# NoSuchThingAsRandom/EpidemicSimulator

Hardware: AMD Instinct MI355X
Metric: citizen-timesteps/sec (higher is better)
Workload: dtype u32 citizen word; u32 uniform vs ceil(q*2^32) (reference: f64 uniform; tolerance 2^-32 per draw); 1 GPU; uk64m: 64000000 citizens, 290000 Output Areas, 10 seeds, steps 1..667 of 5000, interventions on; seed=1592598545

## Files before the change

### epidemicsimulator_amd/csrc/esim_device.h

```cpp
#pragma once
#include <stdint.h>

#define CW_TE_SHIFT    19u
#define CW_BUS_EXPOSED (1u << 18)
#define CW_FLAGS       0xFFu
#define CW_VAX_SHIFT   11u
#define CW_VAX_MASK    (0x7Fu << CW_VAX_SHIFT)
#define CW_KEEP        (CW_FLAGS | CW_VAX_MASK)
#define CW_VAX_NONE    0xFFFFFFFFu
#define CW_PLAN_SKIP   (1u << 10)
#define CW_VAX_REL(w)  ((((w) >> CW_VAX_SHIFT) & 0x7Fu) ? 127u - (((w) >> CW_VAX_SHIFT) & 0x7Fu) : CW_VAX_NONE)
#define CW_VAX_FIELD(j) ((127u - (j)) << CW_VAX_SHIFT)
#define CW_TE(w)       ((w) >> CW_TE_SHIFT)
#define CW_MAKE(te, rest) (((te) << CW_TE_SHIFT) | (rest))
#define TE_SUSCEPTIBLE 0x1FFFu
#define TE_VACCINATED  0x1FFEu
#define TE_RECOVERED   0x1FFDu
#define TE_BIAS        512u
#define TE_SLOTS       8192u
#define ESIM_MAX_STEP  7600u

#define FL_USES_PT        0x01u
#define FL_MASK_COMPLIANT 0x02u
#define FL_SAME_AREA      0x04u
#define FL_WORK_SCHOOL    0x08u
#define FL_HAS_WORK       0x10u
#define FL_BIG_ROUTE      0x20u

#define VACC_BATCH 4096u
#define VACC_WINDOW 32768u
#define VACC_TABLE 16384u
#define VACC_MAX_RATE 8192u
#define NO_ROUTE 0xFFFFFFFFu

#define MARK_SLOTS 4

struct Ctrl {
    uint32_t t;
    uint32_t lockdown;
    uint32_t mask;
    uint32_t vacc_active;
    uint32_t have_elig;
    uint32_t trigger_step;
    uint32_t elig_count;
    uint32_t finished;
    uint32_t stop_when_done;
    uint32_t at_work;
    uint32_t bus_dir;
    uint32_t steps_done;
    uint32_t error;
    uint32_t n_susceptible, n_vaccinated, n_recovered_sentinel;
    uint32_t log_len;
    uint32_t n_touched_bld[MARK_SLOTS], n_touched_room[MARK_SLOTS], n_touched_route[MARK_SLOTS], n_touched_route_big[MARK_SLOTS];
    uint32_t counts[5];
    uint32_t n_riders;
    uint32_t future_t0;
    uint32_t small_done;
    uint32_t chunk_ok;
    uint32_t chunk_t0;
    uint32_t chunk_i0, chunk_i1;
    uint32_t items_per_wave;
    uint32_t chunk_parallel;
    uint32_t chunk_pairs;
    uint32_t n_items;
    uint32_t n_newexp;
    uint32_t n_units, unit_next;
    uint32_t n_route_pairs_big;
    uint32_t chunk_done;
    uint32_t prev_t0, prev_n_items, prev_per_wave;
    uint32_t vax_chunk;
    uint32_t chunk_cut;
    uint32_t prev_cut;
    uint32_t prev_n, prev_n_eff, prev_vax;
    uint32_t vax_cuts;
    uint32_t vax_planned, prev_planned;
    uint32_t xs_need;
    uint32_t xs_need_all;
    uint32_t vax_fail;
    uint32_t err_where;
    uint32_t peer_error;
    uint32_t quiet;
    uint32_t chunk_bus;
    uint32_t replan_from;
    uint32_t repair_ran;
    uint32_t vax_repairs;
};

#define ERR_FIELD(code) ((code) ? 1u << (5u * (((code) < 1u || (code) > 6u ? 6u : (code)) - 1u)) : 0u)
#define ERR_MAX_WORLD 31u
#define XE_WORDS (2u + ERR_MAX_WORLD)
static inline __host__ __device__ uint32_t err_decode(uint32_t word)
{
    for (uint32_t c = 1u; c <= 6u; ++c) if ((word >> (5u * (c - 1u))) & 31u) return c;
    return word ? 6u : 0u;
}

struct UnitRec { uint32_t slot, link, lo, n_mem, code, own, m_first, pad; };

struct BldRec { uint32_t res_lo, res_hi, wrk_lo, wrk_hi, type, ovf_lo, ovf_hi, pad; };
#define SD_REPL 8u

struct ItemRec { uint32_t id, a_lo, a_hi, b_lo, b_hi, aux, link, own; };
#define CHUNK_WAVES_MAX 4096u
#define SLOT_COUNTERS_ONLY 0x40000000u
#ifndef ITEM_RECS
#define ITEM_RECS 7u
#define SLOT_IV_STRIDE 8u
#endif
#define LANE_STATE 24u
#define LANE_HSLOT 25u

struct Decision {
    uint32_t lockdown;
    uint32_t mask;
    uint32_t at_work, bus_dir;
};

struct Dev {
    uint32_t n;
    uint32_t n_global;
    uint32_t id_base;
    uint32_t n_bld, n_room, n_pt;
    uint32_t *cit;
    const uint32_t *home, *work, *room;
    const uint32_t *res_off, *res_idx;
    const uint32_t *wrk_off, *wrk_idx;
    const uint32_t *room_off, *room_idx;
    const uint32_t *room_bld;
    const uint8_t  *bld_type;
    uint32_t *cnt_bld[MARK_SLOTS];
    uint32_t *cnt_room[MARK_SLOTS];
    uint32_t *touched_bld[MARK_SLOTS], *touched_room[MARK_SLOTS], *touched_route[MARK_SLOTS], *touched_route_big[MARK_SLOTS];
    uint32_t *route_flag[MARK_SLOTS];
    uint32_t *exp_step;
    uint32_t *exp_part;
    struct Decision *dec;
    unsigned long long *hkey;
    uint32_t hcap;
    uint32_t *hitems;
    struct ItemRec *item_rec;
    uint32_t *slot_state;
    uint32_t *slot_iv;
    uint32_t *vec;
    uint32_t items_cap;
    struct UnitRec *units;
    uint32_t *route_pairs;
    uint32_t *pair_cnt;
    uint32_t *used_cnt;
    uint32_t *route_pairs_big;
    uint32_t big_pairs_cap;
    const uint32_t *ovf_off;
    uint32_t ovf_room_base;
    uint32_t *ovf;
    uint32_t ovf_n;
    uint32_t n_wrk_idx, n_room_idx;
    const int32_t *sch_of_bld;
    uint32_t n_sch;
    uint32_t *sch_diff;
    const uint4 *where4;
    const struct BldRec *bld8;
    uint32_t *big_list;
    uint32_t big_qcap;
    uint32_t *used_pref;
    uint32_t unit_qcap;
    uint32_t *newexp;
    uint32_t newexp_cap;
    uint32_t *hot;
    uint32_t *cursor;
    uint32_t max_route;
    uint32_t *vax_ev;
    uint32_t *vax_cnt;
    uint32_t *vax_now;
    uint32_t *lost_list;
    uint32_t *vax_delta;
    uint32_t *xf_adj;
    uint32_t *hist;
    uint32_t *log;
    uint32_t *log_off;
    const uint64_t *thr;
    Ctrl *ctrl;
    struct esim_step_result *records;
    uint32_t n_routes;
    const uint32_t *route_off;
    const uint32_t *route_riders;
    const uint32_t *route_of;
    uint32_t *bus_key; uint32_t *bus_idx; uint32_t *bus_cnt; uint8_t *bus_flag;
    uint32_t exposed_time, infected_time, vaccination_rate, bus_capacity, start_hour, end_hour;
    uint32_t seed_lo, seed_hi;
    double thr_lockdown, thr_vacc, thr_mask_pt, thr_mask_all;
    uint32_t max_steps;
    uint32_t n_shards;
    uint32_t n_shared_bld, n_shared_room;
    const int32_t *shared_bld, *shared_room;
    uint32_t *xa, *xb, *xf;
    uint32_t rank, world;
    uint32_t *xv;
    uint32_t *xs;
    uint32_t xs_cap;
    uint32_t *xs_out;
    const uint32_t *shared_mask;
    uint32_t *xc;
    uint32_t *xl;
    uint32_t *xe;
    const int32_t *shared_of_bld, *shared_of_room;
#ifdef ESIM_COUNT_WORK
    unsigned long long *work_cnt;
#endif
#ifdef ESIM_WAVE_PROFILE
    uint32_t *prof_buf;
#endif
    uint32_t xf_n;
    const uint32_t *bld_area;
    uint32_t n_areas;
};

#define XA_HEADER 8u
#define XB_HEADER 8u
#define FREE_MAX 96u
#define HKEY_EMPTY 0xFFFFFFFFFFFFFFFFull
#define PLAN_W 4096u
#define XV_HEADER 8u
#define XS_CAP_MAX (1u << 20)
#define HOT_STRIDE 32u
#define SUBQ 64u
#define HOT_NEWEXP 0u
#define HOT_UNITS 64u
#define HOT_BIGPAIRS 128u
#define HOT_BIG 129u
#define HOT_PREV_NEWEXP 257u
#define HOT_RESET 257u
#define HOT_LOST 321u
#define HOT_COUNT 322u
#define RAISE(ctrl, code, where) do { (ctrl)->error = (uint32_t)(-(code)); (ctrl)->err_where = (where); } while (0)
enum { ERR_AT_BIG_LIST = 2, ERR_AT_ITEM_CHECK = 6, ERR_AT_ROUTE_ITEM = 7, ERR_AT_BIGPAIRS = 10, ERR_AT_SCHOOL = 11 };
#define UNIT_NOOP 0xFFFFFFFFu
#ifndef LOST_CAP
#define LOST_CAP 8192u
#endif
#define CHUNK_BUS_STEPS 32u
#define PAIR_K(per_wave, nbus) ((per_wave) * ((nbus) > 8u ? ((nbus) + 3u) / 4u : 2u))
#define COUNT_GRID 256u
#define EXP_ROWS 32u
#ifndef UNIT_INLINE
#define UNIT_INLINE 1024u
#endif
#ifndef UNIT_PAIRS
#define UNIT_PAIRS 1024u
#endif
#define CHUNK_ROUTE_MAX 2048u
```

### epidemicsimulator_amd/csrc/esim_host_ctx.h

```cpp
namespace {

thread_local std::string g_create_error;

struct Timing {
    bool phase = false, kernel = false;
    uint32_t stride = 16;
    hipEvent_t ev[5] = { nullptr, nullptr, nullptr, nullptr, nullptr };
    double phase_s[3] = { 0, 0, 0 };
    std::vector<hipEvent_t> kev; size_t kev_used = 0;
    hipEvent_t cev[2] = { nullptr, nullptr }; double chunk_ms = 0; uint64_t chunk_steps = 0, chunk_count = 0;
    std::vector<hipEvent_t> pkev; size_t pkev_used = 0; uint64_t pipe_steps = 0;
    hipEvent_t sev[2] = { nullptr, nullptr }; double small_ms = 0; uint64_t small_steps = 0;
    bool kdetail = false;
    std::vector<hipEvent_t> kdev; std::vector<int> kd_kind; size_t kd_used = 0;
    double kd_ms[ESIM_CK_N] = { 0 }; uint64_t kd_calls[ESIM_CK_N] = { 0 };
    bool host_trace = false;
    std::vector<std::pair<const char *, double>> ht;

    static void make_pair(hipEvent_t (&e)[2]) { if (!e[0]) { (void)hipEventCreate(&e[0]); (void)hipEventCreate(&e[1]); } }
    void clear()
    {
        phase_s[0] = phase_s[1] = phase_s[2] = 0;
        kev_used = 0; pkev_used = 0; pipe_steps = 0;
        small_ms = 0; small_steps = 0; chunk_ms = 0; chunk_steps = 0; chunk_count = 0;
    }
    void destroy()
    {
        for (auto &e : ev) if (e) (void)hipEventDestroy(e);
        for (auto &e : cev) if (e) (void)hipEventDestroy(e);
        for (auto &e : sev) if (e) (void)hipEventDestroy(e);
        for (auto *v : { &kev, &pkev, &kdev }) { for (auto &e : *v) (void)hipEventDestroy(e); v->clear(); }
    }
};

struct Comm {
    int rank = 0, world = 1;
    ncclComm_t nccl = nullptr;
    esim_allreduce_fn fn = nullptr; void *user = nullptr;
    std::vector<uint32_t> stage;
    uint32_t *xr = nullptr; size_t xr_n = 0;
    uint64_t chunk_steps = 0, step_steps = 0;
    uint64_t calls = 0;
    double timeout_s = 60.0;
};

struct Pinned {
    Ctrl *ctrl = nullptr;
    esim_step_result *rec = nullptr; size_t rec_n = 0;
    uint32_t first = 0, valid = 0;
    bool track = false;
    bool ctrl_fresh = false;
    uint32_t *area = nullptr; size_t area_n = 0;
    uint32_t *grp = nullptr;
    uint8_t *aw = nullptr;
};

struct RestartStaging {
    uint32_t *seeds_dev = nullptr; size_t seeds_cap = 0;
    struct Block { Ctrl h; uint64_t lut[512]; } *stage = nullptr;
    uint32_t *seeds_stage = nullptr; size_t seeds_stage_n = 0;
    hipEvent_t ev = nullptr; bool ev_used = false;
};

struct Ensemble {
    uint32_t *hit = nullptr, *members = nullptr;
    unsigned long long *sum = nullptr, *sumsq = nullptr;
    int where = ESIM_AREA_HOME; uint32_t mask = 0, min = 0;
    bool arrival = false; uint32_t horizon = 0;
    uint32_t n = 0; bool valid = false;
    enum { ROWS_SERIES = 0, ROWS_SETTINGS = 1, ROWS_REPRODUCTION = 2 };
    struct Rows {
        uint32_t *hit = nullptr, *members = nullptr, *p0 = nullptr, *p1 = nullptr, *occ = nullptr, *vax = nullptr;
        unsigned long long *sum = nullptr, *sumsq = nullptr;
        uint8_t *aw = nullptr;
        int what = 0; uint32_t first = 0, n_rows = 0, stride = 0, min = 0, n_cols = 0;
        bool two = false;
        int kind = ROWS_SERIES;
        uint32_t mask = 0;
        uint32_t r_num = 0, r_den = 0;
        uint32_t *defined = nullptr;
        unsigned long long *sum_o = nullptr, *sumsq_o = nullptr, *cross = nullptr;
    } rows;
    bool series = false;
};

struct Groups {
    uint16_t *lab = nullptr; uint32_t n = 0;
    uint32_t *size = nullptr, *cnt = nullptr;
};

struct Snapshot {
    uint32_t step = 0;
    esim_params P;
    Ctrl h;
    uint32_t *words = nullptr, *hist = nullptr, *log_off = nullptr, *exp_step = nullptr;
    esim_step_result *records = nullptr;
    uint32_t *log = nullptr; size_t log_cap = 0;
    uint32_t last_chunk_pairs = 0; bool quiet = false, repair_armed = false, elig_seen = false;
    uint64_t vax_chunk_steps = 0, vax_chunk_cuts = 0, vax_chunk_repairs = 0;
};

struct Seam { uint32_t step = 0, rate = 0; uint64_t seed = 0; };

struct DrawSeam { uint32_t step = 0; bool twice = false, two_capacities = false; uint64_t seed = 0; double chance = 0.0, mask_effectiveness = 0.0; };

struct Tuning {
    uint32_t grid_citizens = 1, grid_infected = 1, grid_expose = 1;
    uint32_t grid_chunk = 1024;
    bool grid_chunk_env = false;
    bool pipeline = true;
    bool time_parallel = true;
    bool vax_chunks = true;
    bool vax_repair = true;
    bool vax_repair_always = false;
    uint32_t tiny_pairs = 2048;
    uint32_t small_grid = 64, small_mult = 4;
    uint32_t draw_mult = 4, units_mult = 4;
    uint32_t small_max = 128;
    uint32_t pair_log2 = 0;
};

struct PairStats {
    double ms[3] = { 0.0, 0.0, 0.0 };
    uint32_t distinct = 0, capacity = 0, dropped = 0;
};

struct esim_ctx_impl {
    esim_params P;
    Dev d;
    bool uploaded = false;
    hipStream_t stream = nullptr;
    std::string err;
    std::vector<uint32_t> init_state;
    std::vector<uint32_t> init_log;
    size_t cnt_bytes = 0;
    uint32_t *cnt_base = nullptr;
    uint32_t n_routes = 0;
    std::vector<uint32_t> route_tab;
    uint32_t longest_list = 0;
    size_t xa_n = 0, xb_n = 0, xf_n = 0;
    uint64_t pop_hash = 0;
    uint64_t pop_hash_head = 0;
    uint32_t cap_steps = 0;
    uint32_t *area_cnt = nullptr;
    uint32_t *arrival = nullptr;
    std::vector<void *> allocs;
    uint32_t host_t = 1;
    uint32_t last_chunk_pairs = 0;
    uint32_t stop_flag_dev = 0;
    bool quiet = false;
    bool repair_armed = false;
    bool elig_seen = false;
    uint32_t rest_t = 0;
    uint64_t vax_chunk_steps = 0, vax_chunk_cuts = 0, vax_chunk_repairs = 0;
    Timing tm;
    PairStats pair_stats;
    Comm comm;
    Pinned pin;
    RestartStaging rs;
    Ensemble ens;
    Groups grp;
    Snapshot snap;
    Seam seam;
    DrawSeam draw_seam;
    DrawSeam snap_draw_seam;
    Tuning tune;
};

#define CTX(c) (reinterpret_cast<esim_ctx_impl *>(c))

void comm_release(esim_ctx_impl *c);
int wait_stream(esim_ctx_impl *c);

int fail(esim_ctx_impl *c, int code, const std::string &msg)
{
    if (c) c->err = msg; else g_create_error = msg;
    return code;
}

#define HIP_TRY(c, expr)                                                                         \
    do {                                                                                         \
        hipError_t e_ = (expr);                                                                  \
        if (e_ != hipSuccess)                                                                    \
            return fail(c, ESIM_ENODEVICE, std::string(#expr) + ": " + hipGetErrorString(e_));   \
    } while (0)

int alloc_failed(esim_ctx_impl *c, hipError_t e) { return fail(c, ESIM_ENOMEM, std::string("hipMalloc: ") + hipGetErrorString(e)); }

template <class T> int dev_alloc(esim_ctx_impl *c, T **p, size_t n)
{
    void *q = nullptr;
    hipError_t e = hipMalloc(&q, sizeof(T) * (n ? n : 1));
    if (e != hipSuccess) return alloc_failed(c, e);
    c->allocs.push_back(q);
    *p = (T *)q;
    return ESIM_OK;
}

template <class T> int dev_alloc_fill(esim_ctx_impl *c, T **p, size_t n, int byte = 0)
{
    if (int rc = dev_alloc(c, p, n)) return rc;
    if (n) HIP_TRY(c, hipMemset(*p, byte, sizeof(T) * n));
    return ESIM_OK;
}

template <class T> int dev_upload(esim_ctx_impl *c, const T **p, const T *host, size_t n)
{
    T *q = nullptr;
    int rc = dev_alloc(c, &q, n);
    if (rc) return rc;
    if (n) HIP_TRY(c, hipMemcpy(q, host, sizeof(T) * n, hipMemcpyHostToDevice));
    *p = q;
    return ESIM_OK;
}

void free_device(esim_ctx_impl *c)
{
    for (void *p : c->allocs) (void)hipFree(p);
    c->allocs.clear();
    c->uploaded = false;
}

void dev_free(esim_ctx_impl *c, void *p)
{
    auto it = std::find(c->allocs.begin(), c->allocs.end(), p);
    if (it == c->allocs.end()) return;
    c->allocs.erase(it);
    (void)hipFree(p);
}

template <class T> struct DevTmp {
    T *p = nullptr;
    DevTmp() = default; DevTmp(const DevTmp &) = delete; DevTmp &operator=(const DevTmp &) = delete;
    ~DevTmp() { (void)hipFree(p); }
    hipError_t alloc(size_t n) { return hipMalloc((void **)&p, sizeof(T) * std::max<size_t>(1, n)); }
};

int drain(esim_ctx_impl *c) { HIP_TRY(c, hipSetDevice(c->P.device)); HIP_TRY(c, hipStreamSynchronize(c->stream)); return ESIM_OK; }

uint32_t grid_for(size_t items, uint32_t per_block, uint32_t cap)
{
    size_t g = (items + per_block - 1) / per_block;
    return (uint32_t)std::max<size_t>(1, std::min<size_t>(g, cap));
}

static inline void ht_mark(esim_ctx_impl *c, const char *what)
{
    if (!c->tm.host_trace) return;
    timespec ts; clock_gettime(CLOCK_MONOTONIC, &ts);
    c->tm.ht.emplace_back(what, ts.tv_sec * 1e6 + ts.tv_nsec * 1e-3);
}

int read_ctrl(esim_ctx_impl *c, Ctrl *h)
{
    HIP_TRY(c, hipMemcpyAsync(c->pin.ctrl, c->d.ctrl, sizeof(Ctrl), hipMemcpyDeviceToHost, c->stream));
    HIP_TRY(c, hipStreamSynchronize(c->stream));
    *h = *c->pin.ctrl;
    return ESIM_OK;
}

int ctrl_error(esim_ctx_impl *c, const Ctrl &h)
{
    if (!h.error) return ESIM_OK;
    const int code = -(int)(h.peer_error ? err_decode(h.peer_error) : h.error);
    return fail(c, code, "device-side error " + std::to_string(code) + " (S underflow / vaccination window exhausted / a chunk table check; raised at check " +
                         std::to_string(h.err_where) + ", esim_device.h ERR_AT_*)");
}

int device_error(esim_ctx_impl *c)
{
    Ctrl h;
    const int rc = read_ctrl(c, &h);
    return rc ? rc : ctrl_error(c, h);
}

}

extern "C" void esim_default_params(esim_params *p)
{
    if (!p) return;
    p->exposure_chance = 0.00055; p->mask_effectiveness = 0.70;
    p->lockdown_threshold = 0.0034; p->vaccination_threshold = 0.005;
    p->mask_pt_threshold = 0.001; p->mask_everywhere_threshold = 0.0022;
    p->exposed_time = 4 * 24; p->infected_time = 14 * 24;
    p->vaccination_rate = 85 * 18;
    p->bus_capacity = 20;
    p->start_hour = 9; p->end_hour = 17;
    p->seed = 0x5EED2011ull;
    p->device = 0;
    p->max_steps = 5000;
}

extern "C" int esim_threshold_lut(const esim_params *p, uint64_t out[512])
{
    if (!p || !out) return ESIM_EINVAL;
    for (int row = 0; row < 2; ++row) {
        double chance = p->exposure_chance - (row ? p->exposure_chance * p->mask_effectiveness : 0.0) - 0.0;
        if (std::signbit(chance)) chance = 0.0;
        for (int n = 0; n < 256; ++n) {
            const double q = 1.0 - std::pow(1.0 - chance, (double)n);
            const double scaled = std::ceil(std::ldexp(q, 32));
            out[row * 256 + n] = scaled <= 0.0 ? 0ull : (uint64_t)scaled;
        }
    }
    return ESIM_OK;
}

namespace {
int check_params(esim_ctx_impl *c, const esim_params *p, const std::string &who)
{
    if (p->exposed_time + p->infected_time + 2u > TE_BIAS)
        return fail(c, ESIM_ERANGE, who + ": exposed_time + infected_time + 2 exceeds the state encoding (512)");
    if (p->vaccination_rate > VACC_MAX_RATE)
        return fail(c, ESIM_ERANGE, who + ": vaccination_rate above 8192 is not supported");
    if (p->bus_capacity == 0 || p->start_hour == 0 || p->end_hour == 0 || p->start_hour > 24 || p->end_hour > 24)
        return fail(c, ESIM_EINVAL, who + ": bad bus_capacity / working hours");
    {
        const uint32_t h[4] = { (p->start_hour + 23u) % 24u, p->start_hour % 24u, (p->end_hour + 23u) % 24u, p->end_hour % 24u };
        for (int a = 0; a < 4; ++a) for (int b = a + 1; b < 4; ++b)
            if (h[a] == h[b]) return fail(c, ESIM_EINVAL, who + ": start_hour-1, start_hour, end_hour-1, end_hour must be distinct");
        if (p->start_hour > 23 || p->end_hour > 23) return fail(c, ESIM_EINVAL, who + ": working hours must be in 1..23");
    }
    if (p->max_steps == 0 || p->max_steps > ESIM_MAX_STEP)
        return fail(c, ESIM_ERANGE, who + ": max_steps must be in 1..7600");
    if (!(p->exposure_chance >= 0.0 && p->exposure_chance <= 1.0))
        return fail(c, ESIM_EINVAL, who + ": exposure_chance must be a probability");
    return ESIM_OK;
}

void params_to_dev(esim_ctx_impl *c)
{
    Dev &d = c->d;
    d.exposed_time = c->P.exposed_time; d.infected_time = c->P.infected_time;
    d.vaccination_rate = c->P.vaccination_rate; d.bus_capacity = c->P.bus_capacity;
    d.start_hour = c->P.start_hour; d.end_hour = c->P.end_hour;
    d.seed_lo = (uint32_t)c->P.seed; d.seed_hi = (uint32_t)(c->P.seed >> 32);
    d.thr_lockdown = c->P.lockdown_threshold; d.thr_vacc = c->P.vaccination_threshold;
    d.thr_mask_pt = c->P.mask_pt_threshold; d.thr_mask_all = c->P.mask_everywhere_threshold;
    d.max_steps = c->P.max_steps;
    c->xf_n =std::min<uint32_t>(FREE_MAX, c->P.exposed_time + 1u);
    d.xf_n = (uint32_t)c->xf_n;
}
}

extern "C" int esim_create(const esim_params *p, esim_ctx **out)
{
    if (!p || !out) return fail(nullptr, ESIM_EINVAL, "esim_create: null argument");
    if (int rc = check_params(nullptr, p, "esim_create")) return rc;
    int n_dev = 0;
    hipError_t e = hipGetDeviceCount(&n_dev);
    if (e != hipSuccess || n_dev <= 0)
        return fail(nullptr, ESIM_ENODEVICE, std::string("esim_create: no HIP device (") + hipGetErrorString(e) + ")");
    if (p->device < 0 || p->device >= n_dev) return fail(nullptr, ESIM_EINVAL, "esim_create: device ordinal out of range");
    e = hipSetDevice(p->device);
    if (e != hipSuccess) return fail(nullptr, ESIM_ENODEVICE, std::string("hipSetDevice: ") + hipGetErrorString(e));
    esim_ctx_impl *c = new esim_ctx_impl();
    c->P = *p;
    c->cap_steps = p->max_steps;
    if (const char *e = std::getenv("ESIM_COMM_TIMEOUT_S")) { const double v = std::atof(e); if (v > 0.0) c->comm.timeout_s = v; }
    std::memset(&c->d, 0, sizeof c->d);
    e = hipStreamCreateWithFlags(&c->stream, hipStreamNonBlocking);
    if (e != hipSuccess) { delete c; return fail(nullptr, ESIM_ENODEVICE, std::string("hipStreamCreate: ") + hipGetErrorString(e)); }
    for (auto &ev : c->tm.ev) (void)hipEventCreate(&ev);
    *out = reinterpret_cast<esim_ctx *>(c);
    return ESIM_OK;
}

extern "C" void esim_destroy(esim_ctx *ctx)
{
    if (ctx) comm_release(CTX(ctx));
    if (!ctx) return;
    esim_ctx_impl *c = CTX(ctx);
    (void)hipSetDevice(c->P.device);
    if (c->stream) (void)hipStreamSynchronize(c->stream);
    free_device(c);
    c->tm.destroy();
    for (void *p : { (void *)c->pin.ctrl, (void *)c->pin.rec, (void *)c->pin.area, (void *)c->pin.grp, (void *)c->pin.aw, (void *)c->rs.stage, (void *)c->rs.seeds_stage })
        if (p) (void)hipHostFree(p);
    if (c->rs.ev) (void)hipEventDestroy(c->rs.ev);
    if (c->stream) (void)hipStreamDestroy(c->stream);
    delete c;
}

extern "C" const char *esim_last_error(const esim_ctx *ctx)
{
    if (!ctx) return g_create_error.c_str();
    return reinterpret_cast<const esim_ctx_impl *>(ctx)->err.c_str();
}
```

### epidemicsimulator_amd/csrc/esim_host_run.h

```cpp
namespace {

int enqueue_begin(esim_ctx_impl *c, bool time_kernel)
{
    Dev &d = c->d;
    if (c->tm.phase) HIP_TRY(c, hipEventRecord(c->tm.ev[0], c->stream));
    if (time_kernel) HIP_TRY(c, hipEventRecord(c->tm.kev[c->tm.kev_used + 0], c->stream));
    hipLaunchKernelGGL(k_infected, dim3(c->tune.grid_infected), dim3(TPB), 0, c->stream, d);
    if (d.n_shards > 1) {
        const uint32_t n = (uint32_t)std::max<size_t>(XA_HEADER, std::max(d.n_shared_bld, d.n_shared_room));
        hipLaunchKernelGGL(k_pack_a, dim3(grid_for(n, TPB, 1u << 20)), dim3(TPB), 0, c->stream, d);
    }
    if (c->tm.phase) HIP_TRY(c, hipEventRecord(c->tm.ev[1], c->stream));
    return ESIM_OK;
}

int enqueue_exposures(esim_ctx_impl *c)
{
    Dev &d = c->d;
    if (d.n_shards > 1) {
        const uint32_t n = (uint32_t)std::max<size_t>(XA_HEADER, std::max(d.n_shared_bld, d.n_shared_room));
        hipLaunchKernelGGL(k_unpack_a, dim3(grid_for(n, TPB, 1u << 20)), dim3(TPB), 0, c->stream, d);
    }
    hipLaunchKernelGGL(k_expose, dim3(c->tune.grid_expose), dim3(TPB), 0, c->stream, d);
    if (d.n_shards > 1) hipLaunchKernelGGL(k_pack_b, dim3(VACC_WINDOW / TPB), dim3(TPB), 0, c->stream, d);
    if (c->tm.phase) HIP_TRY(c, hipEventRecord(c->tm.ev[2], c->stream));
    return ESIM_OK;
}

int enqueue_finish(esim_ctx_impl *c, bool time_kernel, int mode = -1)
{
    Dev &d = c->d;
    if (mode < 0) mode = d.n_shards > 1 ? 1 : 0;
    hipLaunchKernelGGL(k_finish, dim3(1), dim3(FIN_TPB), 0, c->stream, d, mode);
    if (time_kernel) { HIP_TRY(c, hipEventRecord(c->tm.kev[c->tm.kev_used + 1], c->stream)); c->tm.kev_used += 2; }
    if (c->tm.phase) {
        HIP_TRY(c, hipEventRecord(c->tm.ev[3], c->stream));
        HIP_TRY(c, hipEventSynchronize(c->tm.ev[3]));
        float ms;
        for (int i = 0; i < 3; ++i) { HIP_TRY(c, hipEventElapsedTime(&ms, c->tm.ev[i], c->tm.ev[i + 1])); c->tm.phase_s[i] += ms * 1e-3; }
    }
    c->host_t++;
    HIP_TRY(c, hipGetLastError());
    return ESIM_OK;
}

int check_budget(esim_ctx_impl *c, uint32_t n_steps)
{
    if (!c || !c->uploaded) return fail(c, ESIM_ESTATE, "no population uploaded");
    if ((uint64_t)c->host_t + n_steps - 1 > c->P.max_steps)
        return fail(c, ESIM_ERANGE, "step budget exhausted: max_steps reached (DiseaseModel::max_time_step)");
    return ESIM_OK;
}

bool want_kernel_timing(esim_ctx_impl *c)
{
    Timing &t = c->tm;
    if (!t.kernel || (c->host_t % t.stride) != 0) return false;
    if (t.kev_used + 2 > t.kev.size()) {
        for (int i = 0; i < 2; ++i) { hipEvent_t e; if (hipEventCreate(&e) != hipSuccess) return false; t.kev.push_back(e); }
    }
    return true;
}

void kd_mark(esim_ctx_impl *c, int kind)
{
    Timing &t = c->tm;
    if (!t.kdetail) return;
    if (t.kd_used == t.kdev.size()) { hipEvent_t e; if (hipEventCreate(&e) != hipSuccess) return; t.kdev.push_back(e); t.kd_kind.push_back(0); }
    if (hipEventRecord(t.kdev[t.kd_used], c->stream) != hipSuccess) return;
    t.kd_kind[t.kd_used++] = kind;
}

void kd_resolve(esim_ctx_impl *c)
{
    Timing &t = c->tm;
    for (size_t i = 0; i + 1 < t.kd_used; ++i) {
        if (t.kd_kind[i] >= ESIM_CK_N) continue;
        float ms = 0.f;
        if (hipEventElapsedTime(&ms, t.kdev[i], t.kdev[i + 1]) == hipSuccess) { t.kd_ms[t.kd_kind[i]] += ms; t.kd_calls[t.kd_kind[i]]++; }
    }
    t.kd_used = 0;
}

int chunk_time_begin(esim_ctx_impl *c) { if (c->tm.kernel) { Timing::make_pair(c->tm.cev); HIP_TRY(c, hipEventRecord(c->tm.cev[0], c->stream)); } return ESIM_OK; }
int chunk_time_end(esim_ctx_impl *c) { if (c->tm.kernel) HIP_TRY(c, hipEventRecord(c->tm.cev[1], c->stream)); return ESIM_OK; }

int burst_readback(esim_ctx_impl *c, uint32_t first, uint32_t span, Ctrl *h)
{
    const Dev &d = c->d;
    Pinned &pin = c->pin;
    ht_mark(c, "kernels enqueued");
    HIP_TRY(c, hipMemcpyAsync(pin.ctrl, d.ctrl, sizeof(Ctrl), hipMemcpyDeviceToHost, c->stream));
    const bool rec = pin.track && first == pin.first + pin.valid && (size_t)first + span <= pin.rec_n;
    if (rec) HIP_TRY(c, hipMemcpyAsync(pin.rec + first, d.records + first, sizeof(esim_step_result) * span, hipMemcpyDeviceToHost, c->stream));
    ht_mark(c, "copies enqueued");
    HIP_TRY(c, hipStreamSynchronize(c->stream));
    ht_mark(c, "stream drained");
    *h = *pin.ctrl;
    if (rec && h->t >= first) pin.valid += std::min<uint32_t>(h->t - first, span);
    pin.ctrl_fresh = true;
    if (c->tm.kdetail) kd_resolve(c);
    return ESIM_OK;
}

int run_sequential(esim_ctx_impl *c, uint32_t n_steps, bool allow_early_stop, uint32_t *executed)
{
    Dev &d = c->d; Timing &t = c->tm;
    c->pin.ctrl_fresh = false;
    c->quiet = false;
    uint32_t remaining = n_steps, total = 0; int rc;
    const bool persistent = c->tune.small_max > 0 && !t.phase;
    while (remaining > 0) {
        if (persistent) {
            if (t.kernel) { Timing::make_pair(t.sev); HIP_TRY(c, hipEventRecord(t.sev[0], c->stream)); }
            hipLaunchKernelGGL(k_small, dim3(1), dim3(FIN_TPB), 0, c->stream, d, remaining, c->tune.small_max, 0);
            if (t.kernel) HIP_TRY(c, hipEventRecord(t.sev[1], c->stream));
            Ctrl h;
            if ((rc = read_ctrl(c, &h))) return rc;
            if (t.kernel && h.small_done) { float ms; HIP_TRY(c, hipEventElapsedTime(&ms, t.sev[0], t.sev[1])); t.small_ms += ms; t.small_steps += h.small_done; }
            c->host_t += h.small_done; total += h.small_done; remaining -= h.small_done;
            if ((rc = ctrl_error(c, h))) return rc;
            if (h.finished && allow_early_stop) break;
        }
        if (remaining == 0) break;
        const uint32_t chunk = std::min<uint32_t>(remaining, persistent ? 32u : remaining);
        for (uint32_t s = 0; s < chunk; ++s) {
            const bool tk = want_kernel_timing(c);
            if ((rc = enqueue_begin(c, tk))) return rc;
            if ((rc = enqueue_exposures(c))) return rc;
            if ((rc = enqueue_finish(c, tk, 0))) return rc;
        }
        total += chunk; remaining -= chunk;
    }
    if (executed) *executed = total;
    return ESIM_OK;
}

bool tiny_chunk(const esim_ctx_impl *c) { return c->tune.tiny_pairs && c->last_chunk_pairs <= c->tune.tiny_pairs && c->d.world == 1u && c->d.n_shards == 1u; }
bool small_chunk(const esim_ctx_impl *c) { return c->tune.small_grid && c->last_chunk_pairs < 4096u && c->tune.grid_chunk > c->tune.small_grid && !c->tune.grid_chunk_env; }

struct ChunkPass {
    esim_ctx_impl *c;
    uint32_t limit_t;
    bool kd;
    uint32_t n_ahead() const { return (uint32_t)c->xf_n; }
    void mark(int kind) const { if (kd) kd_mark(c, kind); }
    void future(uint32_t n) const { mark(ESIM_CK_FUTURE); hipLaunchKernelGGL(k_future, dim3(1), dim3(FIN_TPB), 0, c->stream, c->d, n, limit_t); }
    void decide(uint32_t n, int parallel, int vax_in_census) const { mark(ESIM_CK_DECIDE); hipLaunchKernelGGL(k_decide, dim3(1), dim3(64), 0, c->stream, c->d, n, limit_t, parallel, vax_in_census); }
    void vax_plan(int sharded) const { mark(ESIM_CK_VAX); hipLaunchKernelGGL(k_chunk_vax<false>, dim3(FREE_MAX + (sharded ? 0u : 1u)), dim3(FIN_TPB), 0, c->stream, c->d, n_ahead(), limit_t, sharded); }
    void lost() const { mark(ESIM_CK_VAX_REPAIR); hipLaunchKernelGGL(k_chunk_lost, dim3(1), dim3(FIN_TPB), 0, c->stream, c->d); }
    void vax_repair(int sharded) const { hipLaunchKernelGGL(k_chunk_vax<true>, dim3(FREE_MAX), dim3(FIN_TPB), 0, c->stream, c->d, n_ahead(), limit_t, sharded); }
    void front(bool few) const
    {
        const Tuning &t = c->tune;
        const uint32_t g = few ? t.small_grid : t.grid_chunk, g_draw = g * (few ? t.small_mult : t.draw_mult), g_units = g * (few ? t.small_mult : t.units_mult);
        mark(ESIM_CK_MARKS); hipLaunchKernelGGL(k_chunk_marks, dim3(g), dim3(TPB), 0, c->stream, c->d);
        mark(ESIM_CK_FOLD); hipLaunchKernelGGL(k_chunk_fold, dim3(g), dim3(TPB), 0, c->stream, c->d);
        mark(ESIM_CK_DRAW); hipLaunchKernelGGL(k_chunk_draw, dim3(g_draw), dim3(TPB), 0, c->stream, c->d, g * (TPB / 64u));
        mark(ESIM_CK_UNITS); hipLaunchKernelGGL(k_chunk_units, dim3(g_units), dim3(TPB), 0, c->stream, c->d);
    }
    void count() const { mark(ESIM_CK_COUNT); hipLaunchKernelGGL(k_chunk_count, dim3(COUNT_GRID), dim3(TPB), 0, c->stream, c->d); }
    void scatter() const { mark(ESIM_CK_SCATTER); hipLaunchKernelGGL(k_chunk_scatter, dim3(COUNT_GRID), dim3(TPB), 0, c->stream, c->d); }
    void books(int alone, int then_next) const { mark(ESIM_CK_BOOKS); hipLaunchKernelGGL(k_chunk_books, dim3(1), dim3(FIN_TPB), 0, c->stream, c->d, alone, then_next, n_ahead(), limit_t); }
    void vax_final() const { mark(ESIM_CK_VAX_FINAL); hipLaunchKernelGGL(k_chunk_vax_final, dim3(FREE_MAX), dim3(TPB), 0, c->stream, c->d); }
};

void enqueue_parallel_chunk(esim_ctx_impl *c, int then_next, uint32_t limit_t)
{
    const ChunkPass p{ c, limit_t, true };
    const bool alone = c->last_chunk_pairs < 1024u;
    p.front(small_chunk(c));
    if (!alone) p.count();
    p.books(alone ? 1 : 0, then_next);
    if (!alone) p.scatter();
    p.mark(ESIM_CK_N);
}

void enqueue_vax_chunk(esim_ctx_impl *c, uint32_t limit_t)
{
    const ChunkPass p{ c, limit_t, true };
    const Tuning &t = c->tune;
    const bool quiet = c->quiet && c->d.world == 1u;
    p.vax_plan(0);
    p.decide(p.n_ahead(), 1, 0);
    if (!quiet) {
        p.front(small_chunk(c));
        if (c->d.world == 1u && t.vax_repair && (c->repair_armed || t.vax_repair_always)) { p.lost(); p.vax_repair(0); }
    }
    p.count();
    p.books(0, 0);
    if (!quiet) p.scatter();
    p.vax_final();
    p.mark(ESIM_CK_N);
}

void enqueue_free_burst(esim_ctx_impl *c, uint32_t bursts, uint32_t limit_t)
{
    const ChunkPass p{ c, limit_t, true };
    if (tiny_chunk(c)) {
        for (uint32_t g = 0; g < bursts; ++g) {
            p.mark(ESIM_CK_TINY);
            hipLaunchKernelGGL(k_chunk_tiny, dim3(1), dim3(FIN_TPB), 0, c->stream, c->d, g == 0u ? 1 : 0, g + 1u < bursts ? 1 : 0, p.n_ahead(), limit_t);
        }
        p.mark(ESIM_CK_N);
        return;
    }
    p.future(p.n_ahead());
    p.decide(p.n_ahead(), 1, 0);
    for (uint32_t g = 0; g < bursts; ++g) enqueue_parallel_chunk(c, g + 1u < bursts ? 1 : 0, limit_t);
}

int run_chunk(esim_ctx_impl *c, uint32_t n_ahead, uint32_t *executed, Ctrl *state_before)
{
    Dev &d = c->d; Timing &t = c->tm;
    c->pin.ctrl_fresh = false;
    ChunkPass{ c, c->P.max_steps, false }.decide(n_ahead, c->tune.time_parallel ? 1 : 0, 0);
    Ctrl h; int rc;
    if ((rc = read_ctrl(c, &h))) return rc;
    *state_before = h;
    if ((rc = ctrl_error(c, h))) return rc;
    const uint32_t n = h.chunk_ok, t0 = h.t;
    c->last_chunk_pairs = h.chunk_pairs;
    *executed = 0;
    if (n == 0) return ESIM_OK;
    if (h.chunk_parallel) {
        if ((rc = chunk_time_begin(c))) return rc;
        enqueue_parallel_chunk(c, 0, 0u);
        if ((rc = chunk_time_end(c))) return rc;
        if (t.kernel) { float ms; HIP_TRY(c, hipEventSynchronize(t.cev[1])); HIP_TRY(c, hipEventElapsedTime(&ms, t.cev[0], t.cev[1])); t.chunk_ms += ms; }
        HIP_TRY(c, hipGetLastError());
        Ctrl after;
        if ((rc = read_ctrl(c, &after)) || (rc = ctrl_error(c, after))) return rc;
        const uint32_t ran = after.t - t0;
        t.chunk_steps += ran; t.chunk_count += ran ? 1u : 0u;
        *executed = ran;
        return ESIM_OK;
    }
    hipLaunchKernelGGL(k_infected_dec, dim3(c->tune.grid_infected), dim3(TPB), 0, c->stream, d, t0, 0u);
    for (uint32_t j = 0; j < n; ++j) {
        bool tk = t.kernel && ((t0 + j) % t.stride) == 0;
        if (tk && t.pkev_used + 2 > t.pkev.size())
            for (int i = 0; i < 2 && tk; ++i) { hipEvent_t e; if (hipEventCreate(&e) != hipSuccess) tk = false; else t.pkev.push_back(e); }
        if (tk) HIP_TRY(c, hipEventRecord(t.pkev[t.pkev_used], c->stream));
        hipLaunchKernelGGL(k_pipe, dim3(c->tune.grid_expose + c->tune.grid_infected), dim3(TPB), 0, c->stream, d, t0 + j, j, c->tune.grid_expose, j + 1 < n ? 1 : 0);
        if (tk) { HIP_TRY(c, hipEventRecord(t.pkev[t.pkev_used + 1], c->stream)); t.pkev_used += 2; }
    }
    hipLaunchKernelGGL(k_batch_finish, dim3(1), dim3(FIN_TPB), 0, c->stream, d, t0, n);
    HIP_TRY(c, hipGetLastError());
    t.pipe_steps += n;
    *executed = n;
    return ESIM_OK;
}

int run_burst(esim_ctx_impl *c, uint32_t remaining, uint32_t bursts, bool vax, Ctrl *h, uint32_t *done)
{
    const uint32_t first = c->host_t, limit_t = first + remaining - 1u, n_ahead = (uint32_t)c->xf_n;
    int rc;
    if ((rc = chunk_time_begin(c))) return rc;
    if (!vax) enqueue_free_burst(c, bursts, limit_t);
    else for (uint32_t g = 0; g < bursts; ++g) enqueue_vax_chunk(c, limit_t);
    if ((rc = chunk_time_end(c))) return rc;
    if ((rc = burst_readback(c, first, std::min<uint32_t>(remaining, bursts * n_ahead), h))) return rc;
    HIP_TRY(c, hipGetLastError());
    if ((rc = ctrl_error(c, *h))) return rc;
    *done = h->t - first;
    c->last_chunk_pairs = h->chunk_pairs;
    Timing &t = c->tm;
    if (*done && t.kernel) { float ms; HIP_TRY(c, hipEventElapsedTime(&ms, t.cev[0], t.cev[1])); t.chunk_ms += ms; t.chunk_steps += *done; t.chunk_count += (*done + n_ahead - 1u) / n_ahead; }
    c->host_t = h->t;
    return ESIM_OK;
}

int run_steps(esim_ctx_impl *c, uint32_t n_steps, bool allow_early_stop, uint32_t *executed)
{
    Dev &d = c->d;
    const uint32_t n_ahead_max = (uint32_t)c->xf_n;
    uint32_t remaining = n_steps, total = 0; int rc;
    bool stalled = false, probing = false;
    uint32_t backoff = 0, sync_chunks_left = 0;
    const bool vax_ok = c->tune.time_parallel && c->tune.vax_chunks && d.n_shards == 1u;
    bool sequential_only = !c->tune.pipeline || c->tm.phase, vax_regime = vax_ok && c->elig_seen;
    if (c->elig_seen && (!vax_ok || n_steps < 8u)) sequential_only = true;
    auto programme_started = [&]() { c->elig_seen = true; if (vax_ok && remaining >= 8u) vax_regime = true; else sequential_only = true; };
    uint32_t vax_fail = 0;
    while (remaining > 0) {
        c->pin.ctrl_fresh = false;
        if (sequential_only) {
            uint32_t done = 0;
            if ((rc = run_sequential(c, remaining, allow_early_stop, &done))) return rc;
            total += done;
            break;
        }
        if (vax_regime) {
            const uint32_t bursts = vax_fail ? 1u : std::min<uint32_t>((remaining + n_ahead_max - 1u) / n_ahead_max + 1u, 8u);
            Ctrl h;
            uint32_t done = 0;
            if ((rc = run_burst(c, remaining, bursts, true, &h, &done))) return rc;
            c->quiet = h.quiet != 0u;
            if (h.vax_cuts > c->vax_chunk_cuts) c->repair_armed = true;
            c->vax_chunk_steps += done; c->vax_chunk_cuts = h.vax_cuts; c->vax_chunk_repairs = h.vax_repairs;
            total += done; remaining -= done;
            if (h.finished && allow_early_stop) break;
            if (remaining == 0) break;
            if (done) { vax_fail = 0; continue; }
            if (std::getenv("ESIM_DEBUG"))
                std::fprintf(stderr, "[esim] vax burst without progress at t=%u: chunk_ok=%u parallel=%u vax_chunk=%u cut=%u pairs=%u fits_flag=%u elig=%u bursts=%u\n",
                             h.t, h.chunk_ok, h.chunk_parallel, h.vax_chunk, h.chunk_cut, h.chunk_pairs, 0u, h.elig_count, bursts);
            vax_fail = std::min<uint32_t>(vax_fail + 1u, 8u);
            uint32_t seq = 0;
            const uint32_t want = std::min<uint32_t>(remaining, vax_fail <= 1u ? 1u : (vax_fail <= 3u ? 8u : n_ahead_max));
            if ((rc = run_sequential(c, want, allow_early_stop, &seq))) return rc;
            total += seq; remaining -= seq;
            if (seq < want) break;
            continue;
        }
        if (c->tune.time_parallel && !stalled && sync_chunks_left == 0) {
            const uint32_t bursts = std::min<uint32_t>((remaining + n_ahead_max - 1u) / n_ahead_max, probing ? 1u : (small_chunk(c) ? 4u : 16u));
            Ctrl h;
            uint32_t done = 0;
            if ((rc = run_burst(c, remaining, bursts, false, &h, &done))) return rc;
            total += done; remaining -= done;
            if (h.finished) break;
            const bool all = done >= std::min<uint32_t>(remaining + done, bursts * n_ahead_max);
            if (done == 0) { backoff = std::min<uint32_t>(64u, backoff ? backoff * 2u : 1u); sync_chunks_left = backoff; probing = true; }
            else { backoff = 0; probing = !all; }
            if (!all) stalled = true;
            continue;
        }
        stalled = false;
        if (sync_chunks_left) --sync_chunks_left;
        const uint32_t n_ahead = std::min<uint32_t>(remaining, n_ahead_max);
        ChunkPass{ c, c->P.max_steps, false }.future(n_ahead);
        uint32_t done = 0;
        Ctrl before;
        if ((rc = run_chunk(c, n_ahead, &done, &before))) return rc;
        c->host_t = before.t + done; total += done; remaining -= done;
        if (before.finished) break;
        if (done < n_ahead && remaining > 0) {
            if (before.have_elig || before.vacc_active) { programme_started(); continue; }
            uint32_t one = 0;
            if ((rc = run_sequential(c, 1, allow_early_stop, &one))) return rc;
            total += one; remaining -= one;
            if (one == 0) break;
            Ctrl h;
            if ((rc = read_ctrl(c, &h))) return rc;
            if (h.have_elig) programme_started();
        }
        if (allow_early_stop && done > 0) {
            Ctrl h;
            if ((rc = read_ctrl(c, &h))) return rc;
            if (h.finished) { c->host_t = h.t; break; }
        }
    }
    if (executed) *executed = total;
    return ESIM_OK;
}

}

extern "C" int esim_step(esim_ctx *ctx, esim_step_result *out)
{
    esim_ctx_impl *c = CTX(ctx);
    int rc = check_budget(c, 1);
    if (rc) return rc;
    if (c->d.n_shards > 1) return fail(c, ESIM_ESTATE, "esim_step: a sharded population runs with esim_run_sharded");
    HIP_TRY(c, hipSetDevice(c->P.device));
    c->rest_t = 0;
    if ((rc = run_steps(c, 1, false, nullptr))) return rc;
    HIP_TRY(c, hipStreamSynchronize(c->stream));
    if (out) HIP_TRY(c, hipMemcpy(out, &c->d.records[c->host_t - 1], sizeof *out, hipMemcpyDeviceToHost));
    if ((rc = device_error(c))) return rc;
    c->rest_t = c->host_t;
    return ESIM_OK;
}

extern "C" int esim_run(esim_ctx *ctx, uint32_t n_steps, int stop_when_done, esim_step_result *out_array, uint32_t *n_done)
{
    esim_ctx_impl *c = CTX(ctx);
    if (c && c->tm.host_trace) { c->tm.ht.clear(); ht_mark(c, "enter"); }
    int rc = check_budget(c, n_steps);
    if (rc) return rc;
    if (c->d.n_shards > 1) return fail(c, ESIM_ESTATE, "esim_run: a sharded population runs with esim_run_sharded");
    HIP_TRY(c, hipSetDevice(c->P.device));
    Pinned &pin = c->pin;
    const uint32_t first = c->host_t;
    const uint32_t flag = stop_when_done ? 1u : 0u;
    if (flag != c->stop_flag_dev) {
        HIP_TRY(c, hipMemcpyAsync(&c->d.ctrl->stop_when_done, &flag, sizeof flag, hipMemcpyHostToDevice, c->stream));
        HIP_TRY(c, hipStreamSynchronize(c->stream));
        c->stop_flag_dev = flag;
    }
    pin.track = out_array != nullptr; pin.first = first; pin.valid = 0; pin.ctrl_fresh = false;
    c->rest_t = 0;
    rc = run_steps(c, n_steps, stop_when_done != 0, nullptr);
    pin.track = false;
    if (rc) return rc;
    Ctrl h;
    if (pin.ctrl_fresh) h = *pin.ctrl;
    else if ((rc = read_ctrl(c, &h))) return rc;
    if ((rc = ctrl_error(c, h))) return rc;
    const uint32_t done = h.steps_done >= first ? h.steps_done - first + 1 : 0;
    if (std::getenv("ESIM_DEBUG"))
        std::fprintf(stderr, "[esim] esim_run(%u steps from %u): done %u, t=%u steps_done=%u finished=%u chunk_ok=%u parallel=%u, records mirrored %u, control block %s\n",
                     n_steps, first, done, h.t, h.steps_done, h.finished, h.chunk_ok, h.chunk_parallel, pin.valid, pin.ctrl_fresh ? "from the burst" : "read now");
    c->host_t = first + done;
    c->rest_t = c->host_t;
    if (out_array && done) {
        const uint32_t have = std::min(pin.valid, done);
        if (have < done) {
            HIP_TRY(c, hipMemcpyAsync(pin.rec + first + have, c->d.records + first + have, sizeof(esim_step_result) * (done - have), hipMemcpyDeviceToHost, c->stream));
            HIP_TRY(c, hipStreamSynchronize(c->stream));
        }
        std::memcpy(out_array, pin.rec + first, sizeof(esim_step_result) * done);
    }
    if (n_done) *n_done = done;
    if (c->tm.host_trace) {
        ht_mark(c, "exit");
        std::fprintf(stderr, "[esim host trace] esim_run(%u):", n_steps);
        for (size_t i = 1; i < c->tm.ht.size(); ++i) std::fprintf(stderr, " %s +%.1f us;", c->tm.ht[i].first, c->tm.ht[i].second - c->tm.ht[i - 1].second);
        std::fprintf(stderr, " total %.1f us\n", c->tm.ht.back().second - c->tm.ht.front().second);
    }
    return ESIM_OK;
}

extern "C" int esim_set_pipeline(esim_ctx *ctx, int enable)
{
    esim_ctx_impl *c = CTX(ctx); if (!c) return ESIM_EINVAL;
    c->tune.pipeline = enable != 0;
    c->tune.time_parallel = enable >= 2;
    c->tune.vax_chunks = enable >= 3;
    return ESIM_OK;
}

extern "C" int esim_set_small_step_limit(esim_ctx *ctx, uint32_t max_infected)
{
    esim_ctx_impl *c = CTX(ctx); if (!c) return ESIM_EINVAL;
    c->tune.small_max = max_infected;
    return ESIM_OK;
}

extern "C" int esim_set_tiny_chunk_limit(esim_ctx *ctx, uint32_t max_pairs)
{
    esim_ctx_impl *c = CTX(ctx); if (!c) return ESIM_EINVAL;
    c->tune.tiny_pairs = max_pairs;
    return ESIM_OK;
}
```

### epidemicsimulator_amd/csrc/esim_host_upload.h

```cpp
namespace {

struct UploadHost {
    const esim_population *pop;
    uint32_t N, B, R, n_global;
    bool sharded;
    std::vector<uint8_t> fl;
    std::vector<uint32_t> room_fixed;
    std::vector<uint32_t> route_off, riders, route_of;
    uint32_t n_routes = 0, max_route = 0, n_big_routes = 0;
    bool any_big = false;
    std::vector<uint32_t> res_off, res_idx, wrk_off, wrk_idx, room_off, room_idx;
    bool home_sorted = true;
};

int upload_validate(esim_ctx_impl *c, UploadHost &u)
{
    const esim_population *pop = u.pop; const uint32_t N = u.N, B = u.B, R = u.R;
    if (!pop->home_building || !pop->work_building || !pop->room || !pop->flags || !pop->building_area || !pop->building_type)
        return fail(c, ESIM_EINVAL, "esim_upload_population: a required array is NULL");
    if (R && !pop->room_building) return fail(c, ESIM_EINVAL, "esim_upload_population: room_building is NULL");
    if (pop->n_seeds && !pop->seeds) return fail(c, ESIM_EINVAL, "esim_upload_population: seeds is NULL");
    u.n_global = pop->n_citizens_global ? pop->n_citizens_global : N;
    if ((uint64_t)pop->citizen_id_base + N > u.n_global) return fail(c, ESIM_EINVAL, "esim_upload_population: shard range exceeds n_citizens_global");
    u.sharded = u.n_global != N || pop->n_shared_buildings || pop->n_shared_rooms;
    u.fl.resize(N);
    for (uint32_t b = 0; b < B; ++b) {
        if (pop->building_area[b] >= pop->n_areas) return fail(c, ESIM_EINVAL, "esim_upload_population: building_area out of range");
        if (pop->building_type[b] > ESIM_SCHOOL) return fail(c, ESIM_EINVAL, "esim_upload_population: unknown building_type");
    }
    for (uint32_t r = 0; r < R; ++r)
        if (pop->room_building[r] >= B || pop->building_type[pop->room_building[r]] != ESIM_SCHOOL)
            return fail(c, ESIM_EINVAL, "esim_upload_population: room_building must name a School");
    u.room_fixed.assign(N, 0);
    for (uint32_t i = 0; i < N; ++i) {
        const uint32_t hb = pop->home_building[i], wb = pop->work_building[i];
        if (hb >= B || wb >= B) return fail(c, ESIM_EINVAL, "esim_upload_population: building index out of range");
        if (pop->building_type[hb] == ESIM_SCHOOL) return fail(c, ESIM_EINVAL, "esim_upload_population: a School cannot be a home");
        uint8_t f = pop->flags[i] & (FL_USES_PT | FL_MASK_COMPLIANT);
        if (pop->building_area[hb] == pop->building_area[wb]) f |= FL_SAME_AREA;
        if (hb != wb) {
            f |= FL_HAS_WORK;
            if (pop->building_type[wb] == ESIM_SCHOOL) {
                f |= FL_WORK_SCHOOL;
                if (pop->room[i] >= R || pop->room_building[pop->room[i]] != wb)
                    return fail(c, ESIM_EINVAL, "esim_upload_population: school member without a room of that school");
                u.room_fixed[i] = pop->room[i];
            }
        }
        u.fl[i] = f;
    }
    for (uint32_t i = 0; i < pop->n_seeds; ++i)
        if (pop->seeds[i] >= N) return fail(c, ESIM_EINVAL, "esim_upload_population: seed index out of range");
    for (uint32_t i = 0; i < pop->n_shared_buildings; ++i)
        if (pop->shared_building_local[i] >= (int32_t)B) return fail(c, ESIM_EINVAL, "esim_upload_population: shared building out of range");
    for (uint32_t i = 0; i < pop->n_shared_rooms; ++i)
        if (pop->shared_room_local[i] >= (int32_t)R) return fail(c, ESIM_EINVAL, "esim_upload_population: shared room out of range");
    return ESIM_OK;
}

void fnv_mix(uint64_t &h, const void *p, size_t nbytes)
{
    const uint8_t *q = (const uint8_t *)p;
    for (size_t i = 0; i < nbytes; ++i) { h ^= q[i]; h *= 0x100000001b3ull; }
}

uint64_t hash_with_seeds(uint64_t head, const uint32_t *seeds, uint32_t n_seeds)
{
    if (n_seeds) fnv_mix(head, seeds, sizeof(uint32_t) * (size_t)n_seeds);
    return head;
}

uint64_t population_hash(const esim_population *pop, uint64_t *head)
{
    const size_t N = pop->n_citizens, B = pop->n_buildings, R = pop->n_rooms;
    uint64_t h = 0xcbf29ce484222325ull;
    fnv_mix(h, pop->home_building, sizeof(uint32_t) * N); fnv_mix(h, pop->work_building, sizeof(uint32_t) * N);
    fnv_mix(h, pop->room, sizeof(uint32_t) * N); fnv_mix(h, pop->flags, N);
    fnv_mix(h, pop->building_area, sizeof(uint32_t) * B); fnv_mix(h, pop->building_type, B);
    if (R) fnv_mix(h, pop->room_building, sizeof(uint32_t) * R);
    *head = h;
    return hash_with_seeds(h, pop->seeds, pop->n_seeds);
}

void upload_routes(UploadHost &u)
{
    const esim_population *pop = u.pop;
    std::vector<std::pair<uint64_t, uint32_t>> pairs;
    for (uint32_t i = 0; i < u.N; ++i)
        if (u.fl[i] & FL_USES_PT)
            pairs.emplace_back(((uint64_t)pop->building_area[pop->home_building[i]] << 32) | pop->building_area[pop->work_building[i]], i);
    std::sort(pairs.begin(), pairs.end());
    u.riders.resize(pairs.size()); u.route_of.assign(u.N, NO_ROUTE);
    for (size_t i = 0; i < pairs.size(); ++i) {
        if (i == 0 || pairs[i].first != pairs[i - 1].first) u.route_off.push_back((uint32_t)i);
        u.riders[i] = pairs[i].second;
        u.route_of[pairs[i].second] = (uint32_t)u.route_off.size() - 1;
    }
    u.n_routes = (uint32_t)u.route_off.size();
    u.route_off.push_back((uint32_t)pairs.size());
    for (uint32_t r = 0; r < u.n_routes; ++r) {
        const uint32_t sz = u.route_off[r + 1] - u.route_off[r];
        u.max_route = std::max(u.max_route, sz);
        if (sz > 64) { u.any_big = true; ++u.n_big_routes; for (uint32_t q = u.route_off[r]; q < u.route_off[r + 1]; ++q) u.fl[u.riders[q]] |= FL_BIG_ROUTE; }
    }
}

void upload_member_lists(UploadHost &u)
{
    const esim_population *pop = u.pop;
    const std::vector<uint8_t> &fl = u.fl;
    auto csr = [](uint32_t n_keys, uint32_t n_items, auto key_of, auto use, std::vector<uint32_t> &off, std::vector<uint32_t> &idx) {
        off.assign((size_t)n_keys + 1, 0);
        for (uint32_t i = 0; i < n_items; ++i) if (use(i)) off[key_of(i) + 1]++;
        for (uint32_t k = 0; k < n_keys; ++k) off[k + 1] += off[k];
        idx.resize(off[n_keys]);
        std::vector<uint32_t> cur(off.begin(), off.end() - 1);
        for (uint32_t i = 0; i < n_items; ++i) if (use(i)) idx[cur[key_of(i)]++] = i;
    };
    csr(u.B, u.N, [&](uint32_t i) { return pop->home_building[i]; }, [&](uint32_t) { return true; }, u.res_off, u.res_idx);
    for (uint32_t i = 0; i < u.N && u.home_sorted; ++i) u.home_sorted = u.res_idx[i] == i;
    csr(u.B, u.N, [&](uint32_t i) { return pop->work_building[i]; },
        [&](uint32_t i) { return (fl[i] & FL_HAS_WORK) && !(fl[i] & FL_WORK_SCHOOL); }, u.wrk_off, u.wrk_idx);
    csr(u.R, u.N, [&](uint32_t i) { return u.room_fixed[i]; }, [&](uint32_t i) { return (fl[i] & FL_WORK_SCHOOL) != 0; }, u.room_off, u.room_idx);
}

uint32_t seed_te(const esim_ctx_impl *c) { return TE_BIAS - (c->P.exposed_time + 1u); }

int upload_population_tables(esim_ctx_impl *c, const UploadHost &u)
{
    const esim_population *pop = u.pop; const uint32_t N = u.N, B = u.B, R = u.R;
    comm_release(c);
    c->comm.fn = nullptr; c->comm.user = nullptr; c->comm.rank = 0; c->comm.world = 1;
    c->comm.xr = nullptr; c->comm.xr_n = 0;
    free_device(c);
    c->rs.seeds_dev = nullptr; c->rs.seeds_cap = 0;
    c->arrival = nullptr;
    c->ens.hit = c->ens.members = nullptr; c->ens.sum = c->ens.sumsq = nullptr;
    c->ens.rows = Ensemble::Rows(); c->ens.series = false;
    c->ens.valid = false;
    c->grp = Groups();
    c->snap = Snapshot();
    Dev &d = c->d;
    std::memset(&d, 0, sizeof d);
    d.n = N; d.n_global = u.n_global; d.id_base = pop->citizen_id_base; d.n_bld = B; d.n_room = R;
    d.n_pt = (uint32_t)u.riders.size(); d.n_routes = u.n_routes; c->n_routes = u.n_routes;
    d.max_route = u.max_route;
    c->route_tab.assign(3 * (size_t)u.n_routes, 0u);
    for (uint32_t r = 0; r < u.n_routes; ++r) {
        const uint32_t first = u.riders[u.route_off[r]];
        c->route_tab[r] = pop->building_area[pop->home_building[first]];
        c->route_tab[u.n_routes + r] = pop->building_area[pop->work_building[first]];
        c->route_tab[2 * (size_t)u.n_routes + r] = u.route_off[r + 1] - u.route_off[r];
    }
    int rc;
    if ((rc = dev_alloc(c, &d.cit, (size_t)N + 1))) return rc;
    if ((rc = dev_upload(c, &d.home, pop->home_building, N)) || (rc = dev_upload(c, &d.work, pop->work_building, N))) return rc;
    if ((rc = dev_upload(c, &d.room, u.room_fixed.data(), N))) return rc;
    if ((rc = dev_upload(c, &d.res_off, u.res_off.data(), u.res_off.size()))) return rc;
    if (!u.home_sorted) { if ((rc = dev_upload(c, &d.res_idx, u.res_idx.data(), u.res_idx.size()))) return rc; }
    else d.res_idx = nullptr;
    if ((rc = dev_upload(c, &d.wrk_off, u.wrk_off.data(), u.wrk_off.size())) || (rc = dev_upload(c, &d.wrk_idx, u.wrk_idx.data(), u.wrk_idx.size()))) return rc;
    if ((rc = dev_upload(c, &d.room_off, u.room_off.data(), u.room_off.size())) || (rc = dev_upload(c, &d.room_idx, u.room_idx.data(), u.room_idx.size()))) return rc;
    if ((rc = dev_upload(c, &d.room_bld, pop->room_building, R))) return rc;
    if ((rc = dev_upload(c, &d.bld_type, pop->building_type, B))) return rc;
    if ((rc = dev_upload(c, &d.bld_area, pop->building_area, B))) return rc;
    d.n_areas = pop->n_areas;
    if ((rc = dev_alloc(c, &c->area_cnt, (size_t)pop->n_areas * 5u))) return rc;
    const size_t per_parity = (size_t)B + R + u.n_routes;
    if ((rc = dev_alloc(c, &c->cnt_base, MARK_SLOTS * per_parity))) return rc;
    c->cnt_bytes = sizeof(uint32_t) * MARK_SLOTS * per_parity;
    if ((rc = dev_alloc(c, &d.exp_step, 2 * ((size_t)c->cap_steps + 2)))) return rc;
    if ((rc = dev_alloc_fill(c, &d.exp_part, (size_t)EXP_ROWS * 2u * FREE_MAX))) return rc;
    if ((rc = dev_alloc(c, &d.dec, FREE_MAX + 1))) return rc;
    return ESIM_OK;
}

int upload_chunk_tables(esim_ctx_impl *c, const UploadHost &u)
{
    const esim_population *pop = u.pop; const uint32_t N = u.N, B = u.B;
    Dev &d = c->d; int rc;
    uint32_t cap = 1u << 20;
    while (cap < (1u << 26) && cap < N / 2u) cap <<= 1;
    if (const char *e = std::getenv("ESIM_HASH_LOG2")) cap = 1u << std::min(28, std::max(4, std::atoi(e)));
    d.hcap = cap;
    d.items_cap = cap / 4u;
    if ((rc = dev_alloc_fill(c, &d.hkey, cap, 0xFF))) return rc;
    if ((rc = dev_alloc_fill(c, &d.hitems, d.items_cap, 0xFF))) return rc;
    if ((rc = dev_alloc_fill(c, &d.item_rec, d.items_cap))) return rc;
    if ((rc = dev_alloc_fill(c, &d.vec, (size_t)cap * FREE_MAX))) return rc;
    if ((rc = dev_alloc_fill(c, &d.slot_state, cap))) return rc;
    if ((rc = dev_alloc_fill(c, &d.slot_iv, (size_t)cap * SLOT_IV_STRIDE))) return rc;
    size_t units = 0;
    auto add_lists = [&](const std::vector<uint32_t> &off) {
        for (size_t i = 0; i + 1 < off.size(); ++i) {
            const size_t pairs = (size_t)(off[i + 1] - off[i]) * FREE_MAX;
            if (pairs > UNIT_INLINE) units += (pairs + UNIT_PAIRS - 1) / UNIT_PAIRS;
        }
    };
    add_lists(u.res_off); add_lists(u.wrk_off); add_lists(u.room_off);
    units = std::min<size_t>(units, (size_t)N / 8u + 65536u);
    d.unit_qcap = (uint32_t)std::max<size_t>(1024, units * 2u / SUBQ);
    if ((rc = dev_alloc_fill(c, &d.units, (size_t)d.unit_qcap * SUBQ, 0xFF))) return rc;
    if ((rc = dev_alloc_fill(c, &d.route_pairs, (size_t)d.items_cap * (CHUNK_BUS_STEPS / 4u)))) return rc;
    d.big_pairs_cap = (uint32_t)std::max<size_t>(1, std::min<size_t>((size_t)d.items_cap / 4u, u.n_big_routes) * CHUNK_BUS_STEPS);
    if ((rc = dev_alloc_fill(c, &d.route_pairs_big, d.big_pairs_cap))) return rc;
    std::vector<uint32_t> sch_members((size_t)B + 1, 0);
    for (uint32_t i = 0; i < N; ++i) if (u.fl[i] & FL_WORK_SCHOOL) sch_members[pop->work_building[i] + 1]++;
    for (uint32_t b = 0; b < B; ++b) sch_members[b + 1] += sch_members[b];
    std::vector<uint32_t> ovf_off(u.res_off.size());
    for (size_t i = 0; i < u.res_off.size(); ++i) ovf_off[i] = u.res_off[i] + u.wrk_off[i] + sch_members[i];
    if ((rc = dev_upload(c, &d.ovf_off, ovf_off.data(), ovf_off.size()))) return rc;
    c->longest_list = u.max_route;
    for (const std::vector<uint32_t> *off : { &u.res_off, &u.wrk_off, &u.room_off })
        for (size_t i = 1; i < off->size(); ++i) c->longest_list = std::max(c->longest_list, (*off)[i] - (*off)[i - 1]);
    {
        std::vector<int32_t> sch_of(B ? B : 1, -1);
        uint32_t n_sch = 0;
        for (uint32_t b = 0; b < B; ++b) if (pop->building_type[b] == ESIM_SCHOOL) sch_of[b] = (int32_t)n_sch++;
        d.n_sch = n_sch;
        if ((rc = dev_upload(c, &d.sch_of_bld, sch_of.data(), sch_of.size()))) return rc;
    }
    {
        std::vector<uint4> w4(N ? N : 1);
        for (uint32_t i = 0; i < N; ++i) w4[i] = make_uint4(pop->home_building[i], pop->work_building[i], u.room_fixed[i], u.route_of[i]);
        if ((rc = dev_upload(c, &d.where4, w4.data(), w4.size()))) return rc;
        std::vector<BldRec> b8(B ? B : 1);
        for (uint32_t b = 0; b < B; ++b) b8[b] = BldRec{ u.res_off[b], u.res_off[b + 1], u.wrk_off[b], u.wrk_off[b + 1], (uint32_t)pop->building_type[b], ovf_off[b], ovf_off[b + 1], 0u };
        if ((rc = dev_upload(c, &d.bld8, b8.data(), b8.size()))) return rc;
        if ((rc = dev_alloc_fill(c, &d.sch_diff, (size_t)(d.n_sch ? d.n_sch : 1) * SD_REPL * 2u * FREE_MAX))) return rc;
    }
    d.ovf_room_base = ovf_off.back();
    d.ovf_n = d.ovf_room_base + u.room_off.back() + 1u;
    if ((rc = dev_alloc_fill(c, &d.ovf, (size_t)d.ovf_n))) return rc;
    d.n_wrk_idx = (uint32_t)u.wrk_idx.size(); d.n_room_idx = (uint32_t)u.room_idx.size();
    d.big_qcap = d.items_cap / SUBQ;
    if ((rc = dev_alloc_fill(c, &d.big_list, (size_t)d.big_qcap * SUBQ * 3u))) return rc;
    if ((rc = dev_alloc_fill(c, &d.used_pref, CHUNK_WAVES_MAX + 1u))) return rc;
    if ((rc = dev_alloc_fill(c, &d.pair_cnt, 16384u)) || (rc = dev_alloc_fill(c, &d.used_cnt, 16384u))) return rc;
    if ((rc = dev_alloc_fill(c, &d.hot, (size_t)HOT_COUNT * HOT_STRIDE))) return rc;
    d.newexp_cap = N / SUBQ + 1u;
    if ((rc = dev_alloc_fill(c, &d.newexp, (size_t)d.newexp_cap * SUBQ))) return rc;
    if ((rc = dev_alloc_fill(c, &d.cursor, (size_t)EXP_ROWS * FREE_MAX))) return rc;
    return ESIM_OK;
}

int upload_step_tables(esim_ctx_impl *c, const UploadHost &u)
{
    const uint32_t N = u.N, B = u.B, R = u.R;
    Dev &d = c->d; int rc;
    const size_t per_parity = (size_t)B + R + u.n_routes;
    for (int p = 0; p < (int)MARK_SLOTS; ++p) {
        uint32_t *base = c->cnt_base + p * per_parity;
        d.cnt_bld[p] = base; d.cnt_room[p] = base + B; d.route_flag[p] = base + B + R;
        if ((rc = dev_alloc(c, &d.touched_bld[p], B)) || (rc = dev_alloc(c, &d.touched_room[p], R))) return rc;
        if ((rc = dev_alloc(c, &d.touched_route[p], u.n_routes)) || (rc = dev_alloc(c, &d.touched_route_big[p], u.n_routes))) return rc;
    }
    if ((rc = dev_alloc(c, &d.vax_ev, (size_t)FREE_MAX * VACC_MAX_RATE))) return rc;
    if ((rc = dev_alloc_fill(c, &d.vax_cnt, FREE_MAX)) || (rc = dev_alloc_fill(c, &d.vax_now, FREE_MAX))) return rc;
    if ((rc = dev_alloc_fill(c, &d.vax_delta, 4u * (FREE_MAX + 2u)))) return rc;
    if ((rc = dev_alloc_fill(c, &d.lost_list, LOST_CAP))) return rc;
    if ((rc = dev_alloc_fill(c, &d.xf_adj, FREE_MAX + 2u))) return rc;
    if ((rc = dev_alloc(c, &d.hist, TE_SLOTS)) || (rc = dev_alloc(c, &d.log, (size_t)N + 1)) || (rc = dev_alloc(c, &d.log_off, TE_SLOTS + 1))) return rc;
    {
        const uint32_t *sd = nullptr;
        if ((rc = dev_upload(c, &sd, c->init_log.data(), c->init_log.size()))) return rc;
        c->rs.seeds_dev = const_cast<uint32_t *>(sd); c->rs.seeds_cap = c->init_log.size();
    }
    uint64_t lut[512];
    esim_threshold_lut(&c->P, lut);
    if ((rc = dev_upload(c, &d.thr, lut, 512))) return rc;
    if ((rc = dev_alloc(c, &d.ctrl, 1))) return rc;
    if ((rc = dev_alloc(c, &d.records, (size_t)c->cap_steps + 1))) return rc;
    if ((rc = dev_upload(c, &d.route_off, u.route_off.data(), u.route_off.size())) || (rc = dev_upload(c, &d.route_riders, u.riders.data(), u.riders.size()))) return rc;
    if ((rc = dev_upload(c, &d.route_of, u.route_of.data(), N))) return rc;
    const size_t big_scratch = u.any_big ? u.riders.size() : 0;
    if ((rc = dev_alloc(c, &d.bus_key, big_scratch)) || (rc = dev_alloc(c, &d.bus_idx, big_scratch))) return rc;
    if ((rc = dev_alloc(c, &d.bus_cnt, big_scratch)) || (rc = dev_alloc(c, &d.bus_flag, big_scratch))) return rc;
    params_to_dev(c);
    return ESIM_OK;
}

int upload_shard_tables(esim_ctx_impl *c, const UploadHost &u)
{
    const esim_population *pop = u.pop; const uint32_t B = u.B, R = u.R;
    Dev &d = c->d; int rc;
    d.n_shards = u.sharded ? 2u : 1u;
    d.n_shared_bld = pop->n_shared_buildings; d.n_shared_room = pop->n_shared_rooms;
    if ((rc = dev_upload(c, &d.shared_bld, pop->shared_building_local, pop->n_shared_buildings)) || (rc = dev_upload(c, &d.shared_room, pop->shared_room_local, pop->n_shared_rooms))) return rc;
    std::vector<int32_t> of_b(B ? B : 1, -1), of_r(R ? R : 1, -1);
    for (uint32_t i = 0; i < pop->n_shared_buildings; ++i) if (pop->shared_building_local[i] >= 0) of_b[pop->shared_building_local[i]] = (int32_t)i;
    for (uint32_t i = 0; i < pop->n_shared_rooms; ++i) if (pop->shared_room_local[i] >= 0) of_r[pop->shared_room_local[i]] = (int32_t)i;
    if ((rc = dev_upload(c, &d.shared_of_bld, of_b.data(), of_b.size())) || (rc = dev_upload(c, &d.shared_of_room, of_r.data(), of_r.size()))) return rc;
    if ((rc = dev_alloc_fill(c, &d.xv, XV_HEADER + (size_t)FREE_MAX * (PLAN_W / 32u)))) return rc;
    if ((rc = dev_alloc_fill(c, &d.xc, FREE_MAX + 2u)) || (rc = dev_alloc_fill(c, &d.xl, FREE_MAX + 2u)) || (rc = dev_alloc_fill(c, &d.xe, XE_WORDS))) return rc;
    d.rank = 0; d.world = 1; d.xs = nullptr;
#ifdef ESIM_COUNT_WORK
    if ((rc = dev_alloc_fill(c, &d.work_cnt, (size_t)WK_N))) return rc;
#endif
#ifdef ESIM_WAVE_PROFILE
    if ((rc = dev_alloc_fill(c, &d.prof_buf, (size_t)16384 * 16))) return rc;
#endif
    c->xa_n = XA_HEADER + (size_t)d.n_shared_bld + d.n_shared_room;
    c->xb_n = XB_HEADER + VACC_WINDOW / 32u;
    if ((rc = dev_alloc_fill(c, &d.xa, c->xa_n)) || (rc = dev_alloc_fill(c, &d.xb, c->xb_n)) || (rc = dev_alloc_fill(c, &d.xf, FREE_MAX + 1))) return rc;
    return ESIM_OK;
}

template <class T> int pinned_grow(esim_ctx_impl *c, T **p, size_t *have, size_t want)
{
    if (*have >= want) return ESIM_OK;
    if (*p) (void)hipHostFree(*p);
    *p = nullptr; *have = 0;
    HIP_TRY(c, hipHostMalloc((void **)p, sizeof(T) * std::max<size_t>(1, want), hipHostMallocDefault));
    *have = want;
    return ESIM_OK;
}

int upload_pinned(esim_ctx_impl *c, const UploadHost &u)
{
    if (!c->pin.ctrl) HIP_TRY(c, hipHostMalloc((void **)&c->pin.ctrl, sizeof(Ctrl), hipHostMallocDefault));
    if (!c->rs.stage) HIP_TRY(c, hipHostMalloc((void **)&c->rs.stage, sizeof(*c->rs.stage), hipHostMallocDefault));
    if (!c->rs.ev) HIP_TRY(c, hipEventCreateWithFlags(&c->rs.ev, hipEventDisableTiming));
    if (int rc = pinned_grow(c, &c->pin.rec, &c->pin.rec_n, (size_t)c->cap_steps + 1)) return rc;
    return pinned_grow(c, &c->pin.area, &c->pin.area_n, (size_t)u.pop->n_areas * 5u);
}

void upload_tuning(esim_ctx_impl *c, const UploadHost &u)
{
    Tuning &t = c->tune;
    t.grid_citizens = grid_for(u.N, TPB, 2048);
    t.grid_infected = 1024;
    t.grid_expose = 1024;
    if (const char *e = std::getenv("ESIM_GRID_INFECTED")) t.grid_infected = (uint32_t)std::max(1, std::atoi(e));
    const char *gc = std::getenv("ESIM_GRID_CHUNK");
    t.grid_chunk_env = gc != nullptr;
    if (gc) t.grid_chunk = (uint32_t)std::min((int)(CHUNK_WAVES_MAX * 64u / TPB), std::max(16, std::atoi(gc) / 16 * 16));
    if (std::getenv("ESIM_TRACE_HOST")) c->tm.host_trace = true;
    if (const char *e = std::getenv("ESIM_VAX_REPAIR")) { t.vax_repair = std::atoi(e) != 0; t.vax_repair_always = std::atoi(e) >= 2; }
    if (const char *e = std::getenv("ESIM_TINY_PAIRS")) t.tiny_pairs = (uint32_t)std::max(0, std::atoi(e));
    if (const char *e = std::getenv("ESIM_SMALL_GRID")) t.small_grid = (uint32_t)std::max(0, std::atoi(e) / 16 * 16);
    if (const char *e = std::getenv("ESIM_SMALL_MULT")) t.small_mult = (uint32_t)std::min(16, std::max(1, std::atoi(e)));
    if (const char *e = std::getenv("ESIM_DRAW_MULT")) t.draw_mult = (uint32_t)std::min(4, std::max(1, std::atoi(e)));
    if (const char *e = std::getenv("ESIM_UNITS_MULT")) t.units_mult = (uint32_t)std::min(16, std::max(1, std::atoi(e)));
    if (const char *e = std::getenv("ESIM_GRID_EXPOSE")) t.grid_expose = (uint32_t)std::max(1, std::atoi(e));
    t.pair_log2 = 0u;
    if (const char *e = std::getenv("ESIM_PAIR_LOG2")) t.pair_log2 = (uint32_t)std::min(31, std::max(6, std::atoi(e)));
}

}

extern "C" int esim_upload_population(esim_ctx *ctx, const esim_population *pop)
{
    esim_ctx_impl *c = CTX(ctx);
    if (!c || !pop) return fail(c, ESIM_EINVAL, "esim_upload_population: null argument");
    HIP_TRY(c, hipSetDevice(c->P.device));
    UploadHost u;
    u.pop = pop; u.N = pop->n_citizens; u.B = pop->n_buildings; u.R = pop->n_rooms;
    int rc;
    if ((rc = upload_validate(c, u))) return rc;
    c->pop_hash = population_hash(pop, &c->pop_hash_head);
    upload_routes(u);
    upload_member_lists(u);
    c->init_state.resize(u.N);
    for (uint32_t i = 0; i < u.N; ++i) c->init_state[i] = CW_MAKE(TE_SUSCEPTIBLE, (uint32_t)u.fl[i]);
    c->init_log.clear();
    for (uint32_t i = 0; i < pop->n_seeds; ++i) {
        const uint32_t sc = pop->seeds[i];
        if (CW_TE(c->init_state[sc]) != seed_te(c)) { c->init_state[sc] = CW_MAKE(seed_te(c), (uint32_t)u.fl[sc]); c->init_log.push_back(sc); }
    }
    if ((rc = upload_population_tables(c, u))) return rc;
    if ((rc = upload_chunk_tables(c, u))) return rc;
    if ((rc = upload_step_tables(c, u))) return rc;
    if ((rc = upload_shard_tables(c, u))) return rc;
    if ((rc = upload_pinned(c, u))) return rc;
    upload_tuning(c, u);
    c->uploaded = true;
    return esim_reset(ctx);
}

namespace {

void initial_ctrl(const esim_ctx_impl *c, Ctrl *h)
{
    const uint32_t n_seeds = (uint32_t)c->init_log.size();
    std::memset(h, 0, sizeof *h);
    h->t = 1;
    h->mask = ESIM_MASK_NONE;
    h->n_susceptible = c->d.n - n_seeds;
    h->log_len = n_seeds;
}

void rewind_host(esim_ctx_impl *c)
{
    c->host_t = 1;
    c->stop_flag_dev = 0;
    c->last_chunk_pairs = (uint32_t)c->init_log.size();
    c->vax_chunk_steps = 0; c->vax_chunk_cuts = 0; c->elig_seen = false; c->repair_armed = false; c->quiet = false;
    c->pin.track = false; c->pin.ctrl_fresh = false;
    c->rest_t = 0;
    c->seam = Seam();
    c->draw_seam = DrawSeam();
    c->tm.clear();
}

}

extern "C" int esim_reset(esim_ctx *ctx)
{
    esim_ctx_impl *c = CTX(ctx);
    if (!c || !c->uploaded) return fail(c, ESIM_ESTATE, "esim_reset: no population uploaded");
    if (int rc = drain(c)) return rc;
    const Dev &d = c->d;
    const uint32_t n_seeds = (uint32_t)c->init_log.size();
    Ctrl h;
    initial_ctrl(c, &h);
    HIP_TRY(c, hipMemcpy(d.ctrl, &h, sizeof h, hipMemcpyHostToDevice));
    if (d.n) HIP_TRY(c, hipMemcpy(d.cit, c->init_state.data(), sizeof(uint32_t) * (size_t)d.n, hipMemcpyHostToDevice));
    HIP_TRY(c, hipMemset(c->cnt_base, 0, c->cnt_bytes));
    HIP_TRY(c, hipMemset(d.exp_step, 0, sizeof(uint32_t) * 2 * ((size_t)c->P.max_steps + 2)));
    HIP_TRY(c, hipMemset(d.records, 0, sizeof(esim_step_result) * ((size_t)c->P.max_steps + 1)));
    const uint32_t te = seed_te(c);
    std::vector<uint32_t> hist(TE_SLOTS, 0), off(TE_SLOTS + 1, 0);
    hist[te] = n_seeds;
    for (uint32_t k = te + 1; k <= TE_SLOTS; ++k) off[k] = n_seeds;
    HIP_TRY(c, hipMemcpy(d.hist, hist.data(), sizeof(uint32_t) * TE_SLOTS, hipMemcpyHostToDevice));
    HIP_TRY(c, hipMemcpy(d.log_off, off.data(), sizeof(uint32_t) * (TE_SLOTS + 1), hipMemcpyHostToDevice));
    if (n_seeds) HIP_TRY(c, hipMemcpy(d.log, c->init_log.data(), sizeof(uint32_t) * n_seeds, hipMemcpyHostToDevice));
    rewind_host(c);
    return ESIM_OK;
}

namespace {

int restart_check(esim_ctx_impl *c, const esim_params *p, const std::string &who)
{
    if (!c->uploaded) return fail(c, ESIM_ESTATE, who + ": no population uploaded");
    if (c->comm.world > 1) return fail(c, ESIM_ESTATE, who + ": the context has a communicator of several ranks (the shards would have to agree on the parameters)");
    if (int rc = check_params(c, p, who)) return rc;
    if (p->device != c->P.device) return fail(c, ESIM_EINVAL, who + ": device must be the context's device");
    if (p->max_steps > c->cap_steps) return fail(c, ESIM_ERANGE, who + ": max_steps above the max_steps the context was created with (the record log's capacity)");
    return ESIM_OK;
}

int restart_enqueue(esim_ctx_impl *c, const esim_params *p, bool replace, const uint32_t *seeds, uint32_t n_seeds)
{
    HIP_TRY(c, hipSetDevice(c->P.device));
    if (c->rs.ev_used) HIP_TRY(c, hipEventSynchronize(c->rs.ev));
    if (replace) {
        if (int rc = pinned_grow(c, &c->rs.seeds_stage, &c->rs.seeds_stage_n, n_seeds)) return rc;
        if (n_seeds > c->rs.seeds_cap) {
            uint32_t *grown = nullptr;
            if (int rc = dev_alloc(c, &grown, n_seeds)) return rc;
            dev_free(c, c->rs.seeds_dev);
            c->rs.seeds_dev = grown; c->rs.seeds_cap = n_seeds;
        }
    }
    c->P = *p;
    params_to_dev(c);
    const Dev &d = c->d;
    const uint32_t te = seed_te(c);
    if (replace) {
        for (uint32_t sc : c->init_log) c->init_state[sc] = CW_MAKE(TE_SUSCEPTIBLE, c->init_state[sc] & CW_FLAGS);
        c->init_log.clear();
        for (uint32_t i = 0; i < n_seeds; ++i) {
            const uint32_t sc = seeds[i];
            if (CW_TE(c->init_state[sc]) != te) { c->init_state[sc] = CW_MAKE(te, c->init_state[sc] & CW_FLAGS); c->init_log.push_back(sc); }
        }
        c->pop_hash = hash_with_seeds(c->pop_hash_head, seeds, n_seeds);
        c->snap.step = 0;
        if (!c->init_log.empty()) std::memcpy(c->rs.seeds_stage, c->init_log.data(), sizeof(uint32_t) * c->init_log.size());
    } else
        for (uint32_t sc : c->init_log) c->init_state[sc] = CW_MAKE(te, c->init_state[sc] & CW_FLAGS);
    const uint32_t n_seeds_now = (uint32_t)c->init_log.size();
    Ctrl &h = c->rs.stage->h;
    initial_ctrl(c, &h);
    esim_threshold_lut(&c->P, c->rs.stage->lut);
    HIP_TRY(c, hipMemcpyAsync(d.ctrl, &h, sizeof h, hipMemcpyHostToDevice, c->stream));
    HIP_TRY(c, hipMemcpyAsync(const_cast<uint64_t *>(d.thr), c->rs.stage->lut, sizeof c->rs.stage->lut, hipMemcpyHostToDevice, c->stream));
    if (replace && n_seeds_now) HIP_TRY(c, hipMemcpyAsync(c->rs.seeds_dev, c->rs.seeds_stage, sizeof(uint32_t) * n_seeds_now, hipMemcpyHostToDevice, c->stream));
    HIP_TRY(c, hipEventRecord(c->rs.ev, c->stream));
    c->rs.ev_used = true;
    if (d.n) hipLaunchKernelGGL(k_restart_words, dim3(grid_for(((size_t)d.n + 3u) / 4u, TPB, 2048)), dim3(TPB), 0, c->stream, d.cit, d.n);
    HIP_TRY(c, hipMemsetAsync(c->cnt_base, 0, c->cnt_bytes, c->stream));
    HIP_TRY(c, hipMemsetAsync(d.exp_step, 0, sizeof(uint32_t) * 2 * ((size_t)c->cap_steps + 2), c->stream));
    HIP_TRY(c, hipMemsetAsync(d.records, 0, sizeof(esim_step_result) * ((size_t)c->cap_steps + 1), c->stream));
    hipLaunchKernelGGL(k_restart_books, dim3(grid_for(std::max<size_t>(TE_SLOTS + 1u, n_seeds_now), TPB, 0xFFFFFFFFu)), dim3(TPB), 0, c->stream,
                       d.cit, d.n, c->rs.seeds_dev, n_seeds_now, te, d.hist, d.log_off);
    if (n_seeds_now) HIP_TRY(c, hipMemcpyAsync(d.log, c->rs.seeds_dev, sizeof(uint32_t) * n_seeds_now, hipMemcpyDeviceToDevice, c->stream));
    HIP_TRY(c, hipGetLastError());
    rewind_host(c);
    return ESIM_OK;
}

}

extern "C" int esim_restart(esim_ctx *ctx, const esim_params *p)
{
    esim_ctx_impl *c = CTX(ctx);
    if (!c || !p) return fail(c, ESIM_EINVAL, "esim_restart: null argument");
    if (int rc = restart_check(c, p, "esim_restart")) return rc;
    return restart_enqueue(c, p, false, nullptr, 0);
}

extern "C" int esim_restart_seeded(esim_ctx *ctx, const esim_params *p, const uint32_t *seeds, uint32_t n_seeds)
{
    esim_ctx_impl *c = CTX(ctx);
    if (!c || !p) return fail(c, ESIM_EINVAL, "esim_restart_seeded: null argument");
    if (int rc = restart_check(c, p, "esim_restart_seeded")) return rc;
    if (n_seeds && !seeds) return fail(c, ESIM_EINVAL, "esim_restart_seeded: seeds is NULL");
    if (n_seeds > c->d.n) return fail(c, ESIM_ERANGE, "esim_restart_seeded: more seeds than citizens");
    for (uint32_t i = 0; i < n_seeds; ++i)
        if (seeds[i] >= c->d.n) return fail(c, ESIM_EINVAL, "esim_restart_seeded: seed index out of range");
    return restart_enqueue(c, p, true, seeds, n_seeds);
}

extern "C" int esim_get_seeds(esim_ctx *ctx, uint32_t *out, uint32_t cap, uint32_t *n_out)
{
    esim_ctx_impl *c = CTX(ctx);
    if (!c || !n_out) return fail(c, ESIM_EINVAL, "esim_get_seeds: null argument");
    if (!c->uploaded) return fail(c, ESIM_ESTATE, "esim_get_seeds: no population uploaded");
    const uint32_t n = (uint32_t)c->init_log.size();
    *n_out = n;
    if (n > cap || (n && !out)) return fail(c, ESIM_ERANGE, "esim_get_seeds: buffer too small (n_out holds the size needed)");
    if (n) std::memcpy(out, c->init_log.data(), sizeof(uint32_t) * n);
    return ESIM_OK;
}
```

### epidemicsimulator_amd/csrc/esim_kernels_common.h

```cpp
#pragma once
#include <hip/hip_runtime.h>
#include "../../include/esim.h"
#include "esim_device.h"
#include "philox.h"

#define TPB 256
#define FIN_TPB 1024

__device__ __forceinline__ uint32_t status_of(uint32_t te, uint32_t t, uint32_t et, uint32_t it)
{
    if (te == TE_SUSCEPTIBLE) return ESIM_SUSCEPTIBLE;
    if (te == TE_VACCINATED) return ESIM_VACCINATED;
    if (te == TE_RECOVERED) return ESIM_RECOVERED;
    uint32_t d = t + TE_BIAS - te;
    if (d <= et) return ESIM_EXPOSED;
    if (d <= et + 1u + it) return ESIM_INFECTED;
    return ESIM_RECOVERED;
}

__device__ __forceinline__ uint32_t ld(const uint32_t *p)
{
    return __hip_atomic_load(p, __ATOMIC_RELAXED, __HIP_MEMORY_SCOPE_AGENT);
}

__device__ __forceinline__ void schedule(const Dev &d, const Ctrl *ctrl, uint32_t t, uint32_t &at_work, uint32_t &bus_dir)
{
    at_work = ctrl->at_work; bus_dir = ctrl->bus_dir;
    if (ctrl->lockdown) return;
    const uint32_t h = t % 24u;
    if (h == d.start_hour - 1u) bus_dir = 1u;
    else if (h == d.start_hour) { at_work = 1u; bus_dir = 0u; }
    else if (h == d.end_hour - 1u) bus_dir = 2u;
    else if (h == d.end_hour) { at_work = 0u; bus_dir = 0u; }
    else bus_dir = 0u;
}

struct StepEnv { uint32_t t, mask, at_work, bus_dir; };

__device__ __forceinline__ StepEnv env_from_ctrl(const Dev &d, const Ctrl *ctrl)
{
    StepEnv e;
    e.t = ctrl->t; e.mask = ctrl->mask;
    schedule(d, ctrl, e.t, e.at_work, e.bus_dir);
    return e;
}

__device__ __forceinline__ StepEnv env_from_dec(const Dev &d, uint32_t t, uint32_t j)
{
    const Decision q = d.dec[j];
    StepEnv e;
    e.t = t; e.mask = q.mask; e.at_work = q.at_work; e.bus_dir = q.bus_dir;
    return e;
}

__device__ void census_block(const Dev &d, const Ctrl *ctrl, uint32_t t, uint32_t *out )
{
    if (threadIdx.x < 5) out[threadIdx.x] = 0;
    __syncthreads();
    const int hi_e = (int)(t + TE_BIAS);
    const int lo_e = hi_e - (int)d.exposed_time;
    const int hi_i = lo_e - 1;
    const int lo_i = hi_i - (int)d.infected_time;
    uint32_t e = 0, i = 0;
    for (int k = lo_i + (int)threadIdx.x; k <= hi_e; k += (int)blockDim.x) {
        if (k < 0) continue;
        const uint32_t v = ld(&d.hist[k]);
        if (k >= lo_e) e += v; else i += v;
    }
    if (e) atomicAdd(&out[1], e);
    if (i) atomicAdd(&out[2], i);
    __syncthreads();
    if (threadIdx.x == 0) {
        out[0] = ld(&ctrl->n_susceptible); out[4] = ld(&ctrl->n_vaccinated);
        out[3] = d.n - out[0] - out[4] - out[1] - out[2];
    }
    __syncthreads();
}

__device__ __forceinline__ void append(uint32_t *list, uint32_t *len, uint32_t v)
{
    list[atomicAdd(len, 1u)] = v;
}

__device__ __forceinline__ uint32_t steps_ahead(uint32_t t0, uint32_t limit_t, uint32_t max_ahead) { return t0 > limit_t ? 0u : (limit_t - t0 + 1u < max_ahead ? limit_t - t0 + 1u : max_ahead); }

__device__ __forceinline__ void clear_marks(const Dev &d, const Ctrl *ctrl, uint32_t q, uint32_t tid, uint32_t nth)
{
    const uint32_t ob = ctrl->n_touched_bld[q], orr = ctrl->n_touched_room[q], ort = ctrl->n_touched_route[q], orb = ctrl->n_touched_route_big[q];
    for (uint32_t i = tid; i < ob; i += nth) d.cnt_bld[q][d.touched_bld[q][i]] = 0u;
    for (uint32_t i = tid; i < orr; i += nth) d.cnt_room[q][d.touched_room[q][i]] = 0u;
    for (uint32_t i = tid; i < ort; i += nth) d.route_flag[q][d.touched_route[q][i]] = 0u;
    for (uint32_t i = tid; i < orb; i += nth) d.route_flag[q][d.touched_route_big[q][i]] = 0u;
}

__device__ __forceinline__ const uint32_t *newexp_list(const Dev &d, uint32_t r) { return d.newexp + (size_t)r * d.newexp_cap; }
__device__ __forceinline__ uint32_t newexp_len(const Dev &d, uint32_t hot_base, uint32_t r) { return min(ld(&d.hot[(hot_base + r) * HOT_STRIDE]), d.newexp_cap); }

#ifdef ESIM_WAVE_PROFILE
#define PROF_ROW 16u
#define PROF_NOW() ((uint32_t)wall_clock64())
#define PROF_PUT(d, i, v) do { if ((threadIdx.x & 63u) == 0) (d).prof_buf[(size_t)(((blockIdx.x * TPB + threadIdx.x) >> 6)) * PROF_ROW + (i)] = (uint32_t)(v); } while (0)
#define BOOKS_PROF(d, i, v) do { if (threadIdx.x == 0) (d).prof_buf[(size_t)16383 * PROF_ROW + (i)] = (uint32_t)(v); } while (0)
#define TINY_PROF(d, i) do { if (threadIdx.x == 0) (d).prof_buf[(size_t)16382 * PROF_ROW + (i)] = (uint32_t)wall_clock64(); } while (0)
#else
#define BOOKS_PROF(d, i, v) do { (void)sizeof(v); } while (0)
#define TINY_PROF(d, i) do { } while (0)
#define PROF_NOW() 0u
#define PROF_PUT(d, i, v) do { (void)sizeof(v); } while (0)
#endif


#ifdef ESIM_COUNT_WORK
enum { WK_ENTRIES = 0,
       WK_KEYS,
       WK_CLAIMS,
       WK_RECORDS,
       WK_DIRECT,
       WK_FOLDED,
       WK_ITEMS,
       WK_MEMBERS,
       WK_MEMBERS_IDX,
       WK_PAIRS,
       WK_PAIRS_ACTIVE,
       WK_BLOCKS,
       WK_DRAWS,
       WK_UNITS,
       WK_ROUTE_PAIRS,
       WK_RIDERS,
       WK_BUS_DRAWS,
       WK_HITS,
       WK_N };
#define WORK_TALLY uint32_t wk_[WK_N]; for (int wk_i = 0; wk_i < WK_N; ++wk_i) wk_[wk_i] = 0u
#define WORK_ADD(i, x) (wk_[i] += (uint32_t)(x))
#define WORK_FLUSH(d) do { for (int wk_i = 0; wk_i < WK_N; ++wk_i) { uint32_t x_ = wk_[wk_i]; for (int o_ = 32; o_ > 0; o_ >>= 1) x_ += __shfl_xor(x_, o_, 64); \
        if ((threadIdx.x & 63u) == 0 && x_) atomicAdd(&(d).work_cnt[wk_i], (unsigned long long)x_); wk_[wk_i] = 0u; } } while (0)
#define WORK_ARG , uint32_t *wk_
#define WORK_PASS , wk_
#else
#define WORK_TALLY do { } while (0)
#define WORK_ADD(i, x) do { } while (0)
#define WORK_FLUSH(d) do { } while (0)
#define WORK_ARG
#define WORK_PASS
#endif
```

### epidemicsimulator_amd/csrc/esim_kernels_draw.h

```cpp
#pragma once
#include "esim_kernels_common.h"
#include "esim_rank.h"
#include "esim_chunk_sets.h"
#include "esim_kernels_marks.h"
__device__ __forceinline__ void expose_min(const Dev &d, Ctrl *ctrl, uint32_t m, uint32_t w, uint32_t s, uint32_t bus)
{
    const uint32_t cand = CW_MAKE(s + TE_BIAS, bus | (w & CW_KEEP));
    const uint32_t prev = atomicMin(&d.cit[m], cand);
    if (bus && cand < prev && CW_VAX_REL(w) != CW_VAX_NONE) {
        const uint32_t at = atomicAdd(&d.hot[HOT_LOST * HOT_STRIDE], 1u);
        if (at < LOST_CAP) d.lost_list[at] = m;
    }
    if (cand < prev && CW_TE(prev) == TE_SUSCEPTIBLE) {
        const uint32_t r = m & (SUBQ - 1u);
        d.newexp[(size_t)r * d.newexp_cap + atomicAdd(&d.hot[(HOT_NEWEXP + r) * HOT_STRIDE], 1u)] = m;
    }
}

struct ChunkShared {
    Decision dec[FREE_MAX];
    uint64_t thr[512];
};
__device__ __forceinline__ void stage_chunk(const Dev &d, ChunkShared &sm, uint32_t n, uint32_t n_threads)
{
    for (uint32_t i = threadIdx.x; i < n; i += n_threads) sm.dec[i] = d.dec[i];
    for (uint32_t i = threadIdx.x; i < 512u; i += n_threads) sm.thr[i] = d.thr[i];
}
struct RouteShared {
    uint32_t s_key[CHUNK_ROUTE_MAX];
    uint16_t s_bus[CHUNK_ROUTE_MAX];
    uint8_t s_inf[CHUNK_ROUTE_MAX];
    uint32_t s_cnt[CHUNK_ROUTE_MAX + 1];
    uint32_t s_seen[CHUNK_ROUTE_MAX / 32u];
};
#define SLOT_STEPS 4u
struct WaveScratch { uint32_t rounds; uint32_t cnt[FREE_MAX]; uint32_t sch[FREE_MAX]; uint32_t mem_id[64]; uint32_t mem_w[64]; uint4 desc[2u * (FREE_MAX / SLOT_STEPS + 1u)]; };
__device__ __forceinline__ void put_school(WaveScratch &ws, uint32_t lane, uint32_t s0, uint32_t s1) { ws.sch[lane] = s0; if (lane < FREE_MAX - 64u) ws.sch[64u + lane] = s1; }

__device__ __forceinline__ void member_pairs(const Dev &d, Ctrl *ctrl, const ChunkShared &sm, WaveScratch &ws, const uint32_t *idx,
                                             uint32_t lo, uint32_t p_lo, uint32_t p_hi, uint32_t lane, uint32_t kind, uint32_t S, uint32_t t0 WORK_ARG,
                                             bool have_pre = false, uint32_t pre_m = 0u, uint32_t pre_w = 0u, uint32_t pre_base = 0u)
{
    const uint64_t seed = ((uint64_t)d.seed_hi << 32) | d.seed_lo;
    const uint32_t m_first = p_lo / S, m_last = (p_hi - 1u) / S;
    for (uint32_t mb = m_first; mb <= m_last; mb += 64u) {
        __builtin_amdgcn_wave_barrier();
        if (mb + lane <= m_last) {
            WORK_ADD(WK_MEMBERS, 1); WORK_ADD(WK_MEMBERS_IDX, idx ? 1 : 0);
            if (have_pre && mb == pre_base) { ws.mem_id[lane] = pre_m; ws.mem_w[lane] = pre_w; }
            else {
                const uint32_t m = idx ? idx[lo + mb + lane] : lo + mb + lane;
                ws.mem_id[lane] = m;
                ws.mem_w[lane] = d.cit[m];
            }
        }
        __builtin_amdgcn_wave_barrier();
        const uint32_t q_lo = max(p_lo, mb * S), q_hi = min(p_hi, (mb + 64u) * S);
#ifdef ESIM_WAVE_PROFILE
        if (lane == 0) ws.rounds += (q_hi - q_lo + 63u) / 64u;
#endif
        for (uint32_t p = q_lo + lane; p < q_hi; p += 64u) {
            const uint32_t um = p / S, si = p - um * S;
            const uint32_t m = ws.mem_id[um - mb], w = ws.mem_w[um - mb];
            const uint32_t te = CW_TE(w);
            WORK_ADD(WK_PAIRS, 1);
            if (te >= TE_RECOVERED && te != TE_SUSCEPTIBLE) continue;
            const uint4 dsc = ws.desc[2u * si];
            const uint32_t cnt23 = ws.desc[2u * si + 1u].x;
            const int jb = (int)(dsc.x & 127u) - 3;
            const uint32_t mk = (dsc.x >> 8) & 15u, atw = (dsc.x >> 12) & 15u, everywhere = (dsc.x >> 16) & 15u;
            const uint32_t vrel = CW_VAX_REL(w);
            const int js = (int)te + (((w & ~CW_KEEP) & ((1u << CW_TE_SHIFT) - 1u)) ? 1 : 0) - (int)(t0 + TE_BIAS);
            const int lim = min(js, vrel == CW_VAX_NONE ? (int)FREE_MAX : (int)vrel + 1) - jb;
            const uint32_t early = lim <= 0 ? 0u : lim >= (int)SLOT_STEPS ? 15u : (1u << lim) - 1u;
            const bool same = w & FL_SAME_AREA;
            const uint32_t here = kind == 0u ? (((w & FL_HAS_WORK) && !same) ? ~atw : 15u) : (same ? 15u : atw);
            const uint32_t act = mk & early & here;
            if (!act) continue;
            WORK_ADD(WK_PAIRS_ACTIVE, 1);
            const uint32_t nn = kind == 2u ? dsc.z : dsc.y;
            const uint32_t row = (w & FL_MASK_COMPLIANT) ? 0u : everywhere;
            uint64_t thr[SLOT_STEPS];
#pragma unroll
            for (uint32_t h = 0; h < SLOT_STEPS; ++h) thr[h] = sm.thr[(((row >> h) & 1u) << 8) + ((nn >> (8u * h)) & 255u)];
            const uint32_t gid = d.id_base + m;
            const uint32_t s_blk = (uint32_t)((int)t0 + jb) + (uint32_t)__builtin_ctz(act);
            uint32_t hit = 0u;
            if (kind == 2u) {
                const uint32_t cnt[SLOT_STEPS] = { dsc.w & 0xFFFFu, dsc.w >> 16, cnt23 & 0xFFFFu, cnt23 >> 16 };
                uint32_t kmax = 0u;
#pragma unroll
                for (uint32_t h = 0; h < SLOT_STEPS; ++h) if ((act >> h) & 1u) kmax = max(kmax, cnt[h]);
                const uint32_t first_act = act & (0u - act);
#ifdef ESIM_COUNT_WORK
                for (uint32_t h = 0; h < SLOT_STEPS; ++h) if ((act >> h) & 1u) WORK_ADD(WK_DRAWS, cnt[h]);
#endif
                for (uint32_t k = 0; k < kmax && !(hit & first_act); ++k) {
                    WORK_ADD(WK_BLOCKS, 1);
                    const philox_out o = esim_draw_block(seed, gid, s_blk, ESIM_SLOT_ROOM0 + k);
                    const uint32_t wd[SLOT_STEPS] = { o.w0, o.w1, o.w2, o.w3 };
#pragma unroll
                    for (uint32_t h = 0; h < SLOT_STEPS; ++h) if (((act >> h) & 1u) && k < cnt[h] && (uint64_t)wd[h] < thr[h]) hit |= 1u << h;
                }
            } else {
                WORK_ADD(WK_BLOCKS, 1); WORK_ADD(WK_DRAWS, __popc(act));
                const philox_out o = esim_draw_block(seed, gid, s_blk, kind == 0u ? ESIM_SLOT_HOME : ESIM_SLOT_WORK);
                const uint32_t wd[SLOT_STEPS] = { o.w0, o.w1, o.w2, o.w3 };
#pragma unroll
                for (uint32_t h = 0; h < SLOT_STEPS; ++h) if ((uint64_t)wd[h] < thr[h]) hit |= 1u << h;
                hit &= act;
            }
            if (hit) { WORK_ADD(WK_HITS, 1); expose_min(d, ctrl, m, w, (uint32_t)((int)t0 + jb) + (uint32_t)__builtin_ctz(hit), 0u); }
        }
    }
}

__device__ __forceinline__ uint32_t item_steps_regs(uint32_t c0, uint32_t c1, uint32_t lane, WaveScratch &ws, uint32_t t0, const M96 &AW, const M96 &EV)
{
    ws.cnt[lane] = c0;
    if (lane < FREE_MAX - 64u) ws.cnt[64u + lane] = c1;
    const M96 MK = { __ballot(c0 != 0u), (uint32_t)__ballot(lane < FREE_MAX - 64u && c1 != 0u) };
    __builtin_amdgcn_wave_barrier();
    const int j0 = (int)(SLOT_STEPS * lane) - (int)(t0 & (SLOT_STEPS - 1u));
    const uint32_t mk = lane <= FREE_MAX / SLOT_STEPS ? m96_nibble(MK, j0) : 0u;
    const unsigned long long present = __ballot(mk != 0u);
    if (mk) {
        uint32_t c[SLOT_STEPS], sc[SLOT_STEPS];
#pragma unroll
        for (uint32_t h = 0; h < SLOT_STEPS; ++h) {
            const int j = j0 + (int)h;
            const uint32_t jc = (uint32_t)(j < 0 ? 0 : j >= (int)FREE_MAX ? (int)FREE_MAX - 1 : j);
            c[h] = ws.cnt[jc]; sc[h] = ws.sch[jc];
        }
        uint32_t nn = 0u, ns = 0u;
#pragma unroll
        for (uint32_t h = 0; h < SLOT_STEPS; ++h) {
            if (!((mk >> h) & 1u)) c[h] = 0u;
            nn |= (c[h] & 255u) << (8u * h);
            ns |= (sc[h] & 255u) << (8u * h);
        }
        const uint32_t i = (uint32_t)__popcll(present & ((1ull << lane) - 1ull));
        ws.desc[2u * i] = make_uint4((uint32_t)(j0 + 3) | (mk << 8) | (m96_nibble(AW, j0) << 12) | (m96_nibble(EV, j0) << 16), nn, ns,
                                     min(c[0], 0xFFFFu) | (min(c[1], 0xFFFFu) << 16));
        ws.desc[2u * i + 1u] = make_uint4(min(c[2], 0xFFFFu) | (min(c[3], 0xFFFFu) << 16), 0u, 0u, 0u);
    }
    return (uint32_t)__popcll(present);
}

__device__ __forceinline__ void school_counts(const Dev &d, uint32_t s_sch, uint32_t lane, uint32_t n, WaveScratch &ws)
{
    uint32_t c0 = 0u, c1 = 0u;
    if (s_sch != 0xFFFFFFFFu) {
        if (lane < n) c0 = d.vec[(size_t)s_sch * FREE_MAX + lane];
        if (64u + lane < n) c1 = d.vec[(size_t)s_sch * FREE_MAX + 64u + lane];
    }
    put_school(ws, lane, c0, c1);
}

struct UnitSrc { uint32_t slot, link, own; };
__device__ __forceinline__ void list_or_units(const Dev &d, Ctrl *ctrl, const ChunkShared &sm, WaveScratch &ws, const uint32_t *idx,
                                              uint32_t lo, uint32_t hi, const UnitSrc &src, uint32_t lane, uint32_t kind, uint32_t S, uint32_t t0 WORK_ARG,
                                              bool have_pre = false, uint32_t pre_m = 0u, uint32_t pre_w = 0u)
{
    const uint32_t pairs = (hi - lo) * S;
    if (pairs == 0) return;
    if (pairs <= UNIT_INLINE) { member_pairs(d, ctrl, sm, ws, idx, lo, 0u, pairs, lane, kind, S, t0 WORK_PASS, have_pre, pre_m, pre_w); return; }
    const uint32_t n_units = (pairs + UNIT_PAIRS - 1u) / UNIT_PAIRS;
    const uint32_t r = ((blockIdx.x * TPB + threadIdx.x) >> 6) & (SUBQ - 1u);
    uint32_t start = 0;
    if (lane == 0) start = atomicAdd(&d.hot[(HOT_UNITS + r) * HOT_STRIDE], n_units);
    start = __shfl(start, 0, 64);
    UnitRec *q = d.units + (size_t)r * d.unit_qcap;
    if (start + n_units > d.unit_qcap) {
        for (uint32_t i = lane; i < n_units && start + i < d.unit_qcap; i += 64u) q[start + i].code = UNIT_NOOP;
        member_pairs(d, ctrl, sm, ws, idx, lo, 0u, pairs, lane, kind, S, t0 WORK_PASS, have_pre, pre_m, pre_w);
        return;
    }
    for (uint32_t i = lane; i < n_units; i += 64u) {
        const uint32_t p_lo = i * UNIT_PAIRS;
        q[start + i] = UnitRec{ src.slot, kind == 2u ? src.link : 0xFFFFFFFFu, lo, hi - lo, (kind << 30) | p_lo, src.own, p_lo / S, 0u };
    }
}

struct ItemFetch { uint32_t slot, id, a_lo, a_hi, b_lo, b_hi, aux, link, c0, c1; };
__device__ __forceinline__ uint32_t fetch_item(const Dev &d, uint32_t v, uint32_t lane)
{
    uint32_t x = 0u;
    if (lane < 8u) x = reinterpret_cast<const uint32_t *>(d.item_rec)[(size_t)v * 8u + lane];
    else if (lane == LANE_HSLOT) x = d.hitems[v];
    return x;
}
__device__ __forceinline__ uint32_t fetch_slot(const Dev &d, uint32_t slot, uint32_t lane)
{
    uint32_t x = 0u;
    if (slot < d.hcap) {
        if (lane >= 8u && lane < 8u + ITEM_RECS) x = d.slot_iv[(size_t)slot * SLOT_IV_STRIDE + (lane - 8u)];
        else if (lane == LANE_STATE) x = d.slot_state[slot];
    }
    return x;
}
__device__ __forceinline__ uint32_t merge_fetch(uint32_t by_id, uint32_t by_slot, uint32_t lane)
{
    return (lane < 8u || lane == LANE_HSLOT) ? by_id : by_slot;
}

__device__ __forceinline__ void item_counts(const Dev &d, uint32_t x, uint32_t slot, uint32_t lane, uint32_t n, const M96 &AW,
                                            const M96 &BUS, uint32_t &c0, uint32_t &c1)
{
    const uint32_t state = FX(x, LANE_STATE);
    c0 = 0u; c1 = 0u;
    if (state > ITEM_RECS) {
        if (lane < n) c0 = d.vec[(size_t)slot * FREE_MAX + lane];
        if (64u + lane < n) c1 = d.vec[(size_t)slot * FREE_MAX + 64u + lane];
    }
    const uint32_t n_rec = state >= SLOT_COUNTERS_ONLY ? 0u : state < ITEM_RECS ? state : ITEM_RECS;
    for (uint32_t k = 0; k < n_rec; ++k) {
        const uint32_t iv = (uint32_t)__builtin_amdgcn_readlane((int)x, (int)(8u + k));
        iv_count(iv, lane, AW, BUS, c0, c1);
    }
}

__device__ __forceinline__ ItemFetch decode_item(const Dev &d, uint32_t x, uint32_t lane, uint32_t n, const M96 &AW, const M96 &BUS)
{
    ItemFetch f;
    f.slot = FX(x, LANE_HSLOT); f.id = FX(x, 0); f.a_lo = FX(x, 1); f.a_hi = FX(x, 2); f.b_lo = FX(x, 3); f.b_hi = FX(x, 4); f.aux = FX(x, 5); f.link = FX(x, 6);
    f.c0 = 0u; f.c1 = 0u;
    if (f.slot < d.hcap) {
        item_counts(d, x, f.slot, lane, n, AW, BUS, f.c0, f.c1);
        iv_count(FX(x, 7), lane, AW, BUS, f.c0, f.c1);
    }
    return f;
}

__device__ __forceinline__ bool item_ok(const Dev &d, const ItemFetch &it)
{
    if (it.slot >= d.hcap) return false;
    if (it.id < d.n_bld) return it.a_lo <= it.a_hi && it.a_hi <= d.n && it.b_lo <= it.b_hi && it.b_hi <= d.n_wrk_idx;
    if (it.id < d.n_bld + d.n_room) return it.a_lo <= it.a_hi && it.a_hi <= d.n_room_idx && (it.link == 0xFFFFFFFFu || it.link < d.hcap);
    return true;
}
#define PAIR_SPREAD 1237u
__device__ __forceinline__ void route_pair_small(const Dev &d, Ctrl *ctrl, const ChunkShared &sm, uint32_t off, uint32_t sz, uint32_t j, uint32_t t0, uint32_t lane WORK_ARG)
{
    const uint64_t seed = ((uint64_t)d.seed_hi << 32) | d.seed_lo;
    const uint32_t s = t0 + j, mask = sm.dec[j].mask;
    uint32_t c = 0, w = 0, key = 0;
    bool inf = false;
    WORK_ADD(WK_ROUTE_PAIRS, lane == 0 ? 1 : 0); WORK_ADD(WK_RIDERS, lane < sz ? 1 : 0);
    bool can = false;
    if (lane < sz) {
        c = d.route_riders[off + lane];
        w = d.cit[c];
        inf = status_in_chunk(d, w, t0, j) == ESIM_INFECTED;
        can = rider_can(w, s, j);
    }
    if (!__any(inf) || !__any(can)) return;
    const uint32_t cap = d.bus_capacity;
    uint32_t rank = 0;
    if (sz > cap) {
        if (lane < sz) key = philox4x32_10(d.id_base + c, s, ESIM_SLOT_BUS_ORDER, 0u, d.seed_lo, d.seed_hi).w0;
        rank = rank_wave64(key, lane, sz);
    }
    uint32_t bus, n_bus;
    if (cap >= 16u) {
        bus = (rank >= cap ? 1u : 0u) + (rank >= 2u * cap ? 1u : 0u) + (rank >= 3u * cap ? 1u : 0u);
        n_bus = 1u + (sz > cap ? 1u : 0u) + (sz > 2u * cap ? 1u : 0u) + (sz > 3u * cap ? 1u : 0u);
    } else {
        bus = rank / cap;
        n_bus = (sz + cap - 1u) / cap;
    }
    const unsigned long long inf_m = __ballot(inf);
    uint32_t k = 0;
    for (uint32_t b = 0; b < n_bus; ++b) {
        const unsigned long long on_b = __ballot(lane < sz && bus == b);
        if (bus == b) k = (uint32_t)__popcll(on_b & inf_m);
    }
    if (lane < sz && k && can) {
        const uint32_t row = (!(w & FL_MASK_COMPLIANT) && mask == ESIM_MASK_EVERYWHERE) ? 1u : 0u;
        WORK_ADD(WK_BUS_DRAWS, 1);
        if (esim_u32(seed, d.id_base + c, s, ESIM_SLOT_BUS) < sm.thr[row * 256u + (k & 255u)]) { WORK_ADD(WK_HITS, 1); expose_min(d, ctrl, c, w, s, CW_BUS_EXPOSED); }
    }
}
template <uint32_t NT>
__device__ __forceinline__ void route_pair_big(const Dev &d, Ctrl *ctrl, const ChunkShared &sm, RouteShared &rs, uint32_t code, uint32_t t0, uint32_t n WORK_ARG)
{
    const uint64_t seed = ((uint64_t)d.seed_hi << 32) | d.seed_lo;
    const uint32_t r = code >> 7, j = code & 127u;
    if (r >= d.n_routes || j >= n) { if (threadIdx.x == 0) ctrl->error = (uint32_t)(-ESIM_ERANGE); return; }
    const uint32_t off = d.route_off[r], sz = d.route_off[r + 1] - off;
    if (sz > CHUNK_ROUTE_MAX) { if (threadIdx.x == 0) ctrl->error = (uint32_t)(-ESIM_ERANGE); return; }
    const uint32_t s = t0 + j, mask = sm.dec[j].mask;
    WORK_ADD(WK_ROUTE_PAIRS, threadIdx.x == 0 ? 1 : 0);
    int loc_inf = 0, loc_can = 0;
    for (uint32_t i = threadIdx.x; i < sz; i += NT) {
        const uint32_t c = d.route_riders[off + i];
        WORK_ADD(WK_RIDERS, 1);
        const uint32_t w = d.cit[c];
        rs.s_inf[i] = status_in_chunk(d, w, t0, j) == ESIM_INFECTED ? 1 : 0;
        loc_inf |= rs.s_inf[i];
        loc_can |= rider_can(w, s, j) ? 1 : 0;
    }
    const int any_inf = __syncthreads_or(loc_inf), any_can = __syncthreads_or(loc_can);
    if (!any_inf || !any_can) return;
    for (uint32_t i = threadIdx.x; i < sz; i += NT)
        rs.s_key[i] = philox4x32_10(d.id_base + d.route_riders[off + i], s, ESIM_SLOT_BUS_ORDER, 0u, d.seed_lo, d.seed_hi).w0;
    for (uint32_t i = threadIdx.x; i < sz / d.bus_capacity + 1u; i += NT) rs.s_cnt[i] = 0u;
    for (uint32_t i = threadIdx.x; i < (sz + 31u) / 32u; i += NT) rs.s_seen[i] = 0u;
    __syncthreads();
    int tie = 0;
    for (uint32_t i = threadIdx.x; i < sz; i += NT) {
        const uint32_t rank = rank_block(rs.s_key, rs.s_key[i], sz);
        tie |= rank_seen(rs.s_seen, rank) ? 1 : 0;
        const uint32_t bus = rank / d.bus_capacity;
        rs.s_bus[i] = (uint16_t)bus;
        if (rs.s_inf[i]) atomicAdd(&rs.s_cnt[bus], 1u);
    }
    if (__syncthreads_or(tie)) {
        for (uint32_t i = threadIdx.x; i < sz / d.bus_capacity + 1u; i += NT) rs.s_cnt[i] = 0u;
        __syncthreads();
        for (uint32_t i = threadIdx.x; i < sz; i += NT) {
            const uint32_t bus = rank_block_exact(rs.s_key, rs.s_key[i], i, sz) / d.bus_capacity;
            rs.s_bus[i] = (uint16_t)bus;
            if (rs.s_inf[i]) atomicAdd(&rs.s_cnt[bus], 1u);
        }
        __syncthreads();
    }
    for (uint32_t i = threadIdx.x; i < sz; i += NT) {
        const uint32_t k = rs.s_cnt[rs.s_bus[i]];
        if (!k) continue;
        const uint32_t c = d.route_riders[off + i];
        const uint32_t w = d.cit[c];
        if (!rider_can(w, s, j)) continue;
        const uint32_t row = (!(w & FL_MASK_COMPLIANT) && mask == ESIM_MASK_EVERYWHERE) ? 1u : 0u;
        WORK_ADD(WK_BUS_DRAWS, 1);
        if (esim_u32(seed, d.id_base + c, s, ESIM_SLOT_BUS) < sm.thr[row * 256u + (k & 255u)]) { WORK_ADD(WK_HITS, 1); expose_min(d, ctrl, c, w, s, CW_BUS_EXPOSED); }
    }
    __syncthreads();
}

__global__ __launch_bounds__(TPB) void k_chunk_draw(Dev d, uint32_t n_mw)
{
    __shared__ ChunkShared sm;
    __shared__ WaveScratch wsc[TPB / 64];
    Ctrl *ctrl = d.ctrl;
    const uint32_t t0 = ctrl->chunk_t0, n = ctrl->chunk_ok;
    if (!ctrl->chunk_parallel || n == 0u) return;
    const uint32_t lane = threadIdx.x & 63u;
    const uint32_t wave = (blockIdx.x * TPB + threadIdx.x) >> 6, n_waves = (gridDim.x * TPB) >> 6;
    const uint32_t pt0 = PROF_NOW();
    WORK_TALLY;
    uint32_t p_items = 0u, p_item_max = 0u;
    const uint32_t per_wave = ld(&ctrl->items_per_wave);
    if ((unsigned long long)per_wave * n_mw > d.items_cap || n_waves % n_mw != 0u) return;
    const uint32_t G = n_waves / n_mw;
    const uint32_t T = d.used_pref[n_mw];
    const uint32_t coarse = d.used_pref[min(64u * lane, n_mw)];
    const uint32_t Tq = T / n_waves, Tr = T % n_waves;
    const uint32_t d_lo = Tq * wave + (uint32_t)(((unsigned long long)Tr * wave) / n_waves), d_hi = Tq * (wave + 1u) + (uint32_t)(((unsigned long long)Tr * (wave + 1u)) / n_waves);
    uint32_t ow_base = 0u, win = 0u, ow = 0u;
    auto seek = [&](uint32_t i) {
        ow_base = 64u * ((uint32_t)__popcll(__ballot(64u * lane < n_mw && coarse <= i)) - 1u);
        win = d.used_pref[min(ow_base + lane, n_mw)];
        ow = ow_base + (uint32_t)__popcll(__ballot(ow_base + lane < n_mw && win <= i)) - 1u;
    };
    seek(d_lo);
    auto id_of = [&](uint32_t i) -> uint32_t {
        for (;;) {
            const uint32_t rel = ow - ow_base;
            if (rel == 63u) { ow_base = ow; win = d.used_pref[min(ow_base + lane, n_mw)]; continue; }
            if (ow + 1u < n_mw && (uint32_t)__builtin_amdgcn_readlane((int)win, (int)(rel + 1u)) <= i) { ++ow; continue; }
            return ow * per_wave + (i - (uint32_t)__builtin_amdgcn_readlane((int)win, (int)rel));
        }
    };
    uint32_t id_cur = 0u, id_nxt = 0u, sl_cur = 0u;
    if (d_lo < d_hi) id_cur = fetch_item(d, id_of(d_lo), lane);
    if (d_lo + 1u < d_hi) id_nxt = fetch_item(d, id_of(d_lo + 1u), lane);
    const uint32_t K = PAIR_K(per_wave, ld(&ctrl->chunk_bus));
    const uint32_t w_base = wave % n_mw, w_rep = wave / n_mw;
    uint32_t code_l = 0u, off_l = 0u, sz_l = 0u; bool have = false;
    auto deal = [&](uint32_t k0) {
        const uint32_t k = (k0 + lane) * G + w_rep;
        have = false;
        if (k < K) {
            const uint32_t src = (w_base + n_mw - (uint32_t)(((unsigned long long)k * PAIR_SPREAD) % n_mw)) % n_mw;
            code_l = d.route_pairs[(size_t)src * K + k];
            have = k < d.pair_cnt[src] && (code_l >> 7) < d.n_routes && (code_l & 127u) < n;
        }
    };
    auto deal_riders = [&]() { if (have) { const uint32_t r = code_l >> 7; off_l = d.route_off[r]; sz_l = d.route_off[r + 1] - off_l; } };
    deal(0u);
    stage_chunk(d, sm, n, TPB);
    __syncthreads();
    const uint32_t route_base = d.n_bld + d.n_room;
    WaveScratch &ws = wsc[threadIdx.x >> 6];
    const auto [AW, BUS, EV] = chunk_masks(sm.dec, lane, n);
    if (d_lo < d_hi) sl_cur = fetch_slot(d, FX(id_cur, LANE_HSLOT), lane);
    deal_riders();
#ifdef ESIM_WAVE_PROFILE
    if (lane == 0) ws.rounds = 0u;
#endif
    uint32_t pst[5] = { 0u, 0u, 0u, 0u, 0u };
    const uint32_t pt1 = PROF_NOW();
    for (uint32_t v = d_lo; v < d_hi; ++v) {
        const uint32_t x = merge_fetch(id_cur, sl_cur, lane);
        id_cur = id_nxt;
        if (v + 2u < d_hi) id_nxt = fetch_item(d, id_of(v + 2u), lane);
        if (v + 1u < d_hi) sl_cur = fetch_slot(d, FX(id_cur, LANE_HSLOT), lane);
        const uint32_t pq0 = PROF_NOW();
        const ItemFetch it = decode_item(d, x, lane, n, AW, BUS);
        if (it.slot == ITEM_UNUSED) continue;
        if (!item_ok(d, it)) { if (lane == 0) RAISE(ctrl, ESIM_ERANGE, ERR_AT_ITEM_CHECK); continue; }
        if (it.id >= route_base) continue;
        const uint32_t pi0 = PROF_NOW();
        pst[0] += pi0 - pq0;
        (void)pi0; ++p_items; WORK_ADD(WK_ITEMS, lane == 0 ? 1 : 0);
        if (it.id < d.n_bld) {
            if (it.aux == ESIM_SCHOOL) continue;
            const uint32_t n_res = it.a_hi - it.a_lo, n_wrk = it.b_hi - it.b_lo;
            uint32_t rm = 0u, wm = 0u, rw = 0u, ww = 0u;
            if (lane < n_res) rm = d.res_idx ? d.res_idx[it.a_lo + lane] : it.a_lo + lane;
            if (lane < n_wrk) wm = d.wrk_idx[it.b_lo + lane];
            if (lane < n_res) rw = d.cit[rm];
            if (lane < n_wrk) ww = d.cit[wm];
            const uint32_t pq1 = PROF_NOW();
            const uint32_t S = item_steps_regs(it.c0, it.c1, lane, ws, t0, AW, EV);
            __builtin_amdgcn_wave_barrier();
            const uint32_t pq2 = PROF_NOW();
            const UnitSrc src = { it.slot, it.link, FX(x, 7) };
            list_or_units(d, ctrl, sm, ws, d.res_idx, it.a_lo, it.a_hi, src, lane, 0u, S, t0 WORK_PASS, true, rm, rw);
            const uint32_t pq3 = PROF_NOW();
            list_or_units(d, ctrl, sm, ws, d.wrk_idx, it.b_lo, it.b_hi, src, lane, 1u, S, t0 WORK_PASS, true, wm, ww);
            const uint32_t pq4 = PROF_NOW();
            pst[1] += pq1 - pi0; pst[2] += pq2 - pq1; pst[3] += pq3 - pq2; pst[4] += pq4 - pq3;
        } else {
            const uint32_t n_mem = it.a_hi - it.a_lo;
            uint32_t mm = 0u, mw = 0u;
            if (lane < n_mem) mm = d.room_idx[it.a_lo + lane];
            school_counts(d, it.link, lane, n, ws);
            if (lane < n_mem) mw = d.cit[mm];
            const uint32_t S = item_steps_regs(it.c0, it.c1, lane, ws, t0, AW, EV);
            __builtin_amdgcn_wave_barrier();
            const UnitSrc src = { it.slot, it.link, FX(x, 7) };
            list_or_units(d, ctrl, sm, ws, d.room_idx, it.a_lo, it.a_hi, src, lane, 2u, S, t0 WORK_PASS, true, mm, mw);
        }
        __builtin_amdgcn_wave_barrier();
        { const uint32_t dt = PROF_NOW() - pi0; p_item_max = dt > p_item_max ? dt : p_item_max; }
    }
    const uint32_t pt2 = PROF_NOW();
    for (uint32_t k0 = 0; k0 * G < K; k0 += 64u) {
        if (k0) { deal(k0); deal_riders(); }
        unsigned long long todo = __ballot(have);
        while (todo) {
            const int src_lane = __ffsll((long long)todo) - 1;
            todo &= todo - 1ull;
            const uint32_t code = __shfl(code_l, src_lane, 64), off = __shfl(off_l, src_lane, 64), sz = __shfl(sz_l, src_lane, 64);
            route_pair_small(d, ctrl, sm, off, sz, code & 127u, t0, lane WORK_PASS);
        }
    }
    WORK_FLUSH(d);
    const uint32_t pt3 = PROF_NOW();
#ifndef ESIM_PROFILE_UNITS
    PROF_PUT(d, 0, pt0); PROF_PUT(d, 1, pt1); PROF_PUT(d, 2, pt2); PROF_PUT(d, 3, pt3);
    PROF_PUT(d, 4, p_items); PROF_PUT(d, 5, p_item_max); PROF_PUT(d, 6, wsc[threadIdx.x >> 6].rounds);
    PROF_PUT(d, 11, pst[0]); PROF_PUT(d, 12, pst[1]); PROF_PUT(d, 13, pst[2]); PROF_PUT(d, 14, pst[3]); PROF_PUT(d, 15, pst[4]);
#endif
    (void)pst;
    (void)pt0; (void)pt1; (void)pt2; (void)pt3; (void)p_items; (void)p_item_max;
}

__global__ __launch_bounds__(TPB) void k_chunk_units(Dev d)
{
    __shared__ ChunkShared sm;
    __shared__ WaveScratch wsc[TPB / 64];
    __shared__ RouteShared rs;
    Ctrl *ctrl = d.ctrl;
    const uint32_t t0 = ctrl->chunk_t0, n = ctrl->chunk_ok;
    if (!ctrl->chunk_parallel || n == 0u) return;
    const uint32_t lane = threadIdx.x & 63u;
    const uint32_t wave = (blockIdx.x * TPB + threadIdx.x) >> 6, n_waves = (gridDim.x * TPB) >> 6;
    const uint32_t pu0 = PROF_NOW();
    WORK_TALLY;
    uint32_t pu_n = 0u, pu_max = 0u, pu_it = 0u;
    const uint32_t qr = wave & (SUBQ - 1u), first = wave / SUBQ, step = n_waves / SUBQ;
    const uint32_t n_units = step ? min(ld(&d.hot[(HOT_UNITS + qr) * HOT_STRIDE]), d.unit_qcap) : 0u;
    const uint32_t n_pairs = min(ld(&d.hot[HOT_BIGPAIRS * HOT_STRIDE]), d.big_pairs_cap);
    if (__syncthreads_or(first < n_units) == 0 && n_pairs == 0u) return;
    stage_chunk(d, sm, n, TPB);
    __syncthreads();
    WaveScratch &ws = wsc[threadIdx.x >> 6];
    const uint32_t *q_words = reinterpret_cast<const uint32_t *>(d.units + (size_t)qr * d.unit_qcap);
    const auto [AW, BUS, EV] = chunk_masks(sm.dec, lane, n);
    auto unit_words = [&](uint32_t q) -> uint32_t { return lane < 8u ? q_words[(size_t)q * 8u + lane] : 0u; };
    auto member_id = [&](uint32_t u) -> uint32_t {
        const uint32_t code = FX(u, 4), kind = code >> 30, lo = FX(u, 2), n_mem = FX(u, 3), mf = FX(u, 6);
        if (code == UNIT_NOOP || mf + lane >= n_mem) return 0u;
        const uint32_t *idx = kind == 2u ? d.room_idx : kind == 1u ? d.wrk_idx : d.res_idx;
        return idx ? idx[lo + mf + lane] : lo + mf + lane;
    };
    const uint32_t pu1 = PROF_NOW();
    uint32_t u_0 = 0xFFFFFFFFu, u_1 = 0xFFFFFFFFu;
    uint32_t xs_0 = 0u, ys_0 = 0u, mid_0 = 0u;
    if (first < n_units) u_0 = unit_words(first);
    if (first + step < n_units) u_1 = unit_words(first + step);
    if (first < n_units && FX(u_0, 4) != UNIT_NOOP) { xs_0 = fetch_slot(d, FX(u_0, 0), lane); ys_0 = fetch_slot(d, FX(u_0, 1), lane); mid_0 = member_id(u_0); }
    for (uint32_t q = first; q < n_units; q += step) {
        const uint32_t u = u_0, xs = xs_0, ys = ys_0, mid = mid_0;
        u_0 = u_1;
        u_1 = 0xFFFFFFFFu;
        if (q + 2u * step < n_units) u_1 = unit_words(q + 2u * step);
        if (q + step < n_units && FX(u_0, 4) != UNIT_NOOP) { xs_0 = fetch_slot(d, FX(u_0, 0), lane); ys_0 = fetch_slot(d, FX(u_0, 1), lane); mid_0 = member_id(u_0); }
        const uint32_t code = FX(u, 4);
        if (code == UNIT_NOOP) continue;
        const uint32_t pui = PROF_NOW();
        ++pu_n;
        const uint32_t kind = code >> 30, p_lo = code & 0x3FFFFFFFu, slot = FX(u, 0), link = FX(u, 1), lo = FX(u, 2), n_mem = FX(u, 3), own = FX(u, 5), mf = FX(u, 6);
        const uint32_t mw = (mf + lane < n_mem) ? d.cit[mid] : 0u;
        uint32_t c0, c1;
        item_counts(d, xs, slot, lane, n, AW, BUS, c0, c1);
        iv_count(own, lane, AW, BUS, c0, c1);
        if (kind == 2u) {
            uint32_t s0 = 0u, s1 = 0u;
            if (link != 0xFFFFFFFFu) item_counts(d, ys, link, lane, n, AW, BUS, s0, s1);
            put_school(ws, lane, s0, s1);
        }
        const uint32_t *idx = kind == 2u ? d.room_idx : kind == 1u ? d.wrk_idx : d.res_idx;
        const uint32_t S = item_steps_regs(c0, c1, lane, ws, t0, AW, EV);
        __builtin_amdgcn_wave_barrier();
        const uint32_t pairs = n_mem * S;
        WORK_ADD(WK_UNITS, lane == 0 ? 1 : 0);
        member_pairs(d, ctrl, sm, ws, idx, lo, p_lo, min(pairs, p_lo + UNIT_PAIRS), lane, kind, S, t0 WORK_PASS, true, mid, mw, mf);
        __builtin_amdgcn_wave_barrier();
        { const uint32_t dt = PROF_NOW() - pui; pu_max = dt > pu_max ? dt : pu_max; pu_it += (min(pairs, p_lo + UNIT_PAIRS) - p_lo + 63u) / 64u; }
    }
    const uint32_t pu2 = PROF_NOW();
    WORK_FLUSH(d);
#ifdef ESIM_PROFILE_UNITS
    PROF_PUT(d, 0, pu0); PROF_PUT(d, 1, pu1); PROF_PUT(d, 2, pu2); PROF_PUT(d, 4, pu_n); PROF_PUT(d, 5, pu_max); PROF_PUT(d, 7, pu_it);
#endif
    (void)pu0; (void)pu1; (void)pu2; (void)pu_n; (void)pu_max; (void)pu_it;
    for (uint32_t q = blockIdx.x; q < n_pairs; q += gridDim.x) route_pair_big<TPB>(d, ctrl, sm, rs, d.route_pairs_big[q], t0, n WORK_PASS);
    WORK_FLUSH(d);
}
```

### epidemicsimulator_amd/csrc/esim_kernels_marks.h

```cpp
#pragma once
#include "esim_kernels_common.h"
#include "esim_chunk_sets.h"
__device__ __forceinline__ uint32_t hash64(unsigned long long k)
{
    k ^= k >> 33; k *= 0xff51afd7ed558ccdull; k ^= k >> 33; k *= 0xc4ceb9fe1a85ec53ull; k ^= k >> 33;
    return (uint32_t)k;
}

#define ITEM_UNUSED 0xFFFFFFFFu

__global__ __launch_bounds__(TPB) void k_chunk_marks(Dev d)
{
    Ctrl *ctrl = d.ctrl;
    const uint32_t t0 = ctrl->chunk_t0, n = ctrl->chunk_ok;
    if (!ctrl->chunk_parallel || n == 0u) return;
    clear_marks(d, ctrl, (t0 + MARK_SLOTS - 1u) & (MARK_SLOTS - 1u), blockIdx.x * TPB + threadIdx.x, gridDim.x * TPB);
    const uint32_t lane = threadIdx.x & 63u;
    const uint32_t wave = (blockIdx.x * TPB + threadIdx.x) >> 6, n_waves = (gridDim.x * TPB) >> 6;
    const uint32_t i0 = ctrl->chunk_i0, i1 = ctrl->chunk_i1;
    uint32_t n_remote = 0u;
    if (d.world > 1u) for (uint32_t r = 0; r < d.world; ++r) if (r != d.rank) n_remote += min(d.xs[(size_t)r * (1u + 3u * d.xs_cap)], d.xs_cap);
    const uint32_t per_wave = 4u * ((i1 - i0 + n_remote + n_waves - 1u) / n_waves + (n_remote ? 1u : 0u));
    if (wave == 0 && lane == 0) { ctrl->items_per_wave = per_wave; ctrl->n_items = per_wave * n_waves; }
    if ((unsigned long long)per_wave * n_waves > d.items_cap) { if (lane == 0) ctrl->error = (uint32_t)(-ESIM_ERANGE); return; }
    uint32_t next_id = wave * per_wave;
    const ChunkMasks cm = chunk_masks(d.dec, lane, n);
    const M96 &AW = cm.AW, &BUS = cm.BUS;
    const unsigned long long lt = (1ull << lane) - 1ull;
    const uint32_t pm0 = PROF_NOW();
    WORK_TALLY;
    uint32_t p_entries = 0u;
    uint32_t my_pairs = 0u;
    uint32_t ps[5] = { 0u, 0u, 0u, 0u, 0u };
    const uint32_t E = i1 - i0, total = E + n_remote;
    for (uint32_t round = 0; wave + n_waves * (round * 64u) < total; ++round) {
        const uint32_t pa = PROF_NOW();
        const uint32_t idx = wave + n_waves * (round * 64u + lane);
        bool act = idx < total;
        const bool remote = act && idx >= E;
        uint32_t c = 0u, w = 0u, r_bld = 0xFFFFFFFFu, r_room = 0xFFFFFFFFu;
        if (act && !remote) { c = d.log[i0 + idx]; w = d.cit[c]; }
        if (remote) {
            uint32_t e = idx - E;
            const uint32_t *seg = nullptr;
            for (uint32_t r = 0; r < d.world; ++r) {
                if (r == d.rank) continue;
                const uint32_t *sg = d.xs + (size_t)r * (1u + 3u * d.xs_cap);
                const uint32_t cnt = min(sg[0], d.xs_cap);
                if (e < cnt) { seg = sg; break; }
                e -= cnt;
            }
            act = false;
            if (seg) {
                w = seg[1u + 3u * e];
                const uint32_t sb = seg[2u + 3u * e], sr = seg[3u + 3u * e];
                const int32_t lb = d.shared_bld[sb];
                if (lb >= 0) {
                    act = true;
                    r_bld = (uint32_t)lb;
                    const int32_t lr = sr != 0xFFFFFFFFu ? d.shared_room[sr] : -1;
                    if (lr >= 0) r_room = (uint32_t)lr;
                }
            }
        }
        const Stretch st = infected_stretch(d, w, t0, n, AW, BUS, act);
        const bool any_home = !remote && m96_any(st.home), any_work = m96_any(st.work), any_bus = !remote && m96_any(st.bus);
        const bool school = w & FL_WORK_SCHOOL;
        if (any_home || any_work || any_bus) { ++p_entries; WORK_ADD(WK_ENTRIES, 1); }
        uint32_t src[4] = { 0u, r_bld, r_room, 0u };
        if (!remote && (any_home || any_work || any_bus)) {
            const uint4 k4 = d.where4[c];
            src[0] = k4.x; src[1] = k4.y; src[2] = k4.z; src[3] = k4.w;
        }
        unsigned long long key[4];
        key[0] = any_home ? (unsigned long long)src[0] : HKEY_EMPTY;
        key[1] = any_work ? (unsigned long long)src[1] : HKEY_EMPTY;
        key[2] = (any_work && school && src[2] != 0xFFFFFFFFu) ? (unsigned long long)d.n_bld + src[2] : HKEY_EMPTY;
        key[3] = any_bus ? (unsigned long long)d.n_bld + d.n_room + src[3] : HKEY_EMPTY;
        const uint32_t pb = PROF_NOW() + (uint32_t)(key[0] & 0ull) + (uint32_t)(key[1] & 0ull) + (uint32_t)(key[2] & 0ull) + (uint32_t)(key[3] & 0ull);
        uint32_t slot[4];
        unsigned long long seen[4];
#pragma unroll
        for (uint32_t k = 0; k < 4u; ++k) {
            slot[k] = hash64(key[k]) & (d.hcap - 1u);
            seen[k] = key[k];
            if (key[k] != HKEY_EMPTY) seen[k] = d.hkey[slot[k]];
        }
#pragma unroll
        for (uint32_t k = 0; k < 4u; ++k)
            if (key[k] != HKEY_EMPTY && seen[k] == HKEY_EMPTY) seen[k] = atomicCAS(&d.hkey[slot[k]], HKEY_EMPTY, key[k]);
        bool claimed[4], pending[4];
#pragma unroll
        for (uint32_t k = 0; k < 4u; ++k) {
            claimed[k] = false; pending[k] = false;
            if (key[k] == HKEY_EMPTY) continue;
            WORK_ADD(WK_KEYS, 1);
            if (seen[k] == HKEY_EMPTY) claimed[k] = true;
            else if (seen[k] == key[k]) pending[k] = true;
            else {
                uint32_t h = slot[k];
                bool found = false;
                for (uint32_t probe = 1; probe < d.hcap && !found; ++probe) {
                    h = (h + 1u) & (d.hcap - 1u);
                    const unsigned long long old = atomicCAS(&d.hkey[h], HKEY_EMPTY, key[k]);
                    if (old == HKEY_EMPTY) { claimed[k] = true; found = true; }
                    else if (old == key[k]) { pending[k] = true; found = true; }
                }
                if (!found) { ctrl->error = (uint32_t)(-ESIM_ERANGE); key[k] = HKEY_EMPTY; h = 0u; }
                slot[k] = h;
            }
        }
        const uint32_t pc = PROF_NOW() + (slot[0] & 0u) + (slot[1] & 0u) + (slot[2] & 0u) + (slot[3] & 0u);
        const uint32_t iv_home = stretch_record(st, w);
        const uint32_t iv_work = iv_home | IV_AS_WORK;
        uint32_t before = 0u, n_claims = 0u;
#pragma unroll
        for (uint32_t k = 0; k < 4u; ++k) { const unsigned long long cm = __ballot(claimed[k]); before += (uint32_t)__popcll(cm & lt); n_claims += (uint32_t)__popcll(cm); }
#pragma unroll
        for (uint32_t k = 0; k < 4u; ++k) {
            if (claimed[k]) {
                WORK_ADD(WK_CLAIMS, 1);
                const uint32_t v = next_id + before++;
                d.hitems[v] = slot[k];
                const uint32_t id = (uint32_t)key[k];
                ItemRec rec = { id, 0u, 0u, 0u, 0u, 0u, k == 2u ? slot[1] : 0xFFFFFFFFu,
                                k == 0u ? iv_home : (k == 1u && !school) || k == 2u ? iv_work : 0u };
                if (k == 0u || k == 1u) {
                    const uint4 b4 = *reinterpret_cast<const uint4 *>(&d.bld8[id]);
                    rec.a_lo = b4.x; rec.a_hi = b4.y; rec.b_lo = b4.z; rec.b_hi = b4.w;
                    rec.aux = d.bld8[id].type;
                } else if (k == 2u) {
                    const uint32_t r = id - d.n_bld;
                    rec.a_lo = d.room_off[r]; rec.a_hi = d.room_off[r + 1u];
                    rec.aux = d.room_bld[r];
                }
                d.item_rec[v] = rec;
            }
        }
        next_id += n_claims;
        const uint32_t pd = PROF_NOW();
        uint32_t mine = 0u;
        if (any_bus) {
            uint32_t i = 0u;
            for (unsigned long long m = BUS.lo; m; m &= m - 1ull, ++i) mine |= (uint32_t)((st.bus.lo >> __builtin_ctzll(m)) & 1ull) << i;
            for (uint32_t m = BUS.hi; m; m &= m - 1u, ++i) mine |= ((st.bus.hi >> __builtin_ctz(m)) & 1u) << i;
        }
        bool add_rec[3];
        uint32_t old[4] = { 0u, 0u, 0u, 0u };
#pragma unroll
        for (uint32_t k = 0; k < 3u; ++k) {
            add_rec[k] = pending[k] && !(k == 1u && school);
            if (add_rec[k]) old[k] = atomicAdd(&d.slot_state[slot[k]], 1u);
        }
        if (claimed[1] && school) d.slot_state[slot[1]] = SLOT_COUNTERS_ONLY;
        if (any_bus && key[3] != HKEY_EMPTY) old[3] = atomicOr(&d.slot_state[slot[3]], mine);
        bool direct[3], first[3];
        uint32_t first_base[3] = { 0u, 0u, 0u }, first_cap[3] = { 0u, 0u, 0u };
        if (school && key[1] != HKEY_EMPTY) {
            const int32_t sch = d.sch_of_bld[(uint32_t)key[1]];
            if (sch < 0 || (uint32_t)sch >= d.n_sch) RAISE(ctrl, ESIM_ERANGE, ERR_AT_SCHOOL);
            else {
                uint32_t *dd = d.sch_diff + ((size_t)sch * SD_REPL + (wave & (SD_REPL - 1u))) * 2u * FREE_MAX;
                WORK_ADD(WK_DIRECT, (w & FL_USES_PT) ? 4 : 2);
                atomicAdd(&dd[st.iv_a], 1u);
                if (st.iv_b + 1u < FREE_MAX) atomicAdd(&dd[st.iv_b + 1u], 0xFFFFFFFFu);
                if (w & FL_USES_PT) {
                    atomicAdd(&dd[FREE_MAX + st.iv_a], 1u);
                    if (st.iv_b + 1u < FREE_MAX) atomicAdd(&dd[FREE_MAX + st.iv_b + 1u], 0xFFFFFFFFu);
                }
                if (claimed[1]) { first_base[1] = (uint32_t)sch; first_cap[1] = 0xFFFFFFFFu; }
            }
        }
#pragma unroll
        for (uint32_t k = 0; k < 3u; ++k) {
            direct[k] = false; first[k] = k == 1u && first_cap[1] == 0xFFFFFFFFu;
            if (!add_rec[k]) continue;
            WORK_ADD(WK_RECORDS, 1);
            const uint32_t iv = k == 0u ? iv_home : iv_work;
            if (old[k] < ITEM_RECS) { d.slot_iv[(size_t)slot[k] * SLOT_IV_STRIDE + old[k]] = iv; continue; }
            const uint32_t q = old[k] - ITEM_RECS, id = (uint32_t)key[k];
            uint32_t base, cap;
            if (k < 2u) { base = d.bld8[id].ovf_lo; cap = d.bld8[id].ovf_hi - base; }
            else { const uint32_t r = id - d.n_bld; const uint32_t o = d.room_off[r]; base = d.ovf_room_base + o; cap = d.room_off[r + 1u] - o; }
            if (q < cap) { d.ovf[base + q] = iv; first[k] = q == 0u; first_base[k] = base; first_cap[k] = cap; }
            else direct[k] = true;
        }
        {
            const unsigned long long f[3] = { __ballot(first[0]), __ballot(first[1]), __ballot(first[2]) };
            const uint32_t n_first = (uint32_t)(__popcll(f[0]) + __popcll(f[1]) + __popcll(f[2]));
            if (n_first) {
                const uint32_t r = wave & (SUBQ - 1u);
                uint32_t at0 = 0u;
                if (lane == 0) at0 = atomicAdd(&d.hot[(HOT_BIG + r) * HOT_STRIDE], n_first);
                at0 = __shfl(at0, 0, 64);
                uint32_t *bl = d.big_list + (size_t)r * d.big_qcap * 3u;
                uint32_t at = at0;
#pragma unroll
                for (uint32_t k = 0; k < 3u; ++k) {
                    const uint32_t pos = at + (uint32_t)__popcll(f[k] & lt);
                    if (first[k] && pos < d.big_qcap) { bl[3u * pos] = slot[k]; bl[3u * pos + 1u] = first_base[k]; bl[3u * pos + 2u] = first_cap[k]; }
                    at += (uint32_t)__popcll(f[k]);
                }
                if (at0 + n_first > d.big_qcap && lane == 0) ctrl->error = (uint32_t)(-ESIM_ERANGE);
            }
        }
#pragma unroll
        for (uint32_t k = 0; k < 3u; ++k) {
            const M96 at = k == 0u ? st.home : st.work;
            for (unsigned long long sp = __ballot(direct[k]); sp; sp &= sp - 1ull) {
                const int src_lane = __builtin_ctzll(sp);
                const uint32_t sl = __shfl(slot[k], src_lane, 64), hi = __shfl(at.hi, src_lane, 64);
                const unsigned long long lo = ((unsigned long long)__shfl((uint32_t)(at.lo >> 32), src_lane, 64) << 32) | __shfl((uint32_t)at.lo, src_lane, 64);
                uint32_t *v = d.vec + (size_t)sl * FREE_MAX;
                WORK_ADD(WK_DIRECT, ((lo >> lane) & 1ull) + ((lane < 32u && ((hi >> lane) & 1u)) ? 1 : 0));
                if ((lo >> lane) & 1ull) atomicAdd(&v[lane], 1u);
                if (lane < 32u && ((hi >> lane) & 1u)) atomicAdd(&v[64u + lane], 1u);
            }
        }
        const uint32_t pe = PROF_NOW() + (old[0] & 0u) + (old[1] & 0u) + (old[2] & 0u) + (old[3] & 0u);
        const uint32_t new_bits = (any_bus && key[3] != HKEY_EMPTY) ? (mine & ~old[3]) : 0u;
        if (__any(new_bits != 0u)) {
            const bool big = w & FL_BIG_ROUTE;
            const uint32_t rt = src[3];
            const uint32_t K = PAIR_K(per_wave, ctrl->chunk_bus);
            uint32_t *list = d.route_pairs + (size_t)wave * K;
            uint32_t n_big = 0u;
            for (uint32_t i = 0; i < CHUNK_BUS_STEPS; ++i) n_big += (uint32_t)__popcll(__ballot(big && ((new_bits >> i) & 1u)));
            uint32_t big_base = 0u;
            if (n_big) {
                if (lane == 0) big_base = atomicAdd(&d.hot[HOT_BIGPAIRS * HOT_STRIDE], n_big);
                big_base = __shfl(big_base, 0, 64);
                if (big_base + n_big > d.big_pairs_cap) { if (lane == 0) ctrl->error = (uint32_t)(-ESIM_ERANGE); n_big = 0u; big_base = 0xFFFFFFFFu; }
            }
            uint32_t i = 0u;
            auto put = [&](uint32_t j) {
                const bool f = (new_bits >> i) & 1u;
                const unsigned long long ms = __ballot(f && !big), mb = __ballot(f && big);
                if (f && !big) {
                    const uint32_t pos = my_pairs + (uint32_t)__popcll(ms & lt);
                    if (pos < K) list[pos] = (rt << 7) | j; else ctrl->error = (uint32_t)(-ESIM_ERANGE);
                }
                if (f && big && big_base != 0xFFFFFFFFu) d.route_pairs_big[big_base + (uint32_t)__popcll(mb & lt)] = (rt << 7) | j;
                my_pairs += (uint32_t)__popcll(ms);
                if (big_base != 0xFFFFFFFFu) big_base += (uint32_t)__popcll(mb);
                ++i;
            };
            for (unsigned long long m = BUS.lo; m; m &= m - 1ull) put((uint32_t)__builtin_ctzll(m));
            for (uint32_t m = BUS.hi; m; m &= m - 1u) put(64u + (uint32_t)__builtin_ctz(m));
            my_pairs = min(my_pairs, K);
        }
        { const uint32_t pf = PROF_NOW(); ps[0] += pb - pa; ps[1] += pc - pb; ps[2] += pd - pc; ps[3] += pe - pd; ps[4] += pf - pe; }
    }
    if (lane == 0) { d.pair_cnt[wave] = my_pairs; d.used_cnt[wave] = next_id - wave * per_wave; }
    WORK_FLUSH(d);
    const uint32_t pm1 = PROF_NOW();
    PROF_PUT(d, 8, pm0); PROF_PUT(d, 9, pm1); PROF_PUT(d, 10, p_entries);
    PROF_PUT(d, 11, ps[0]); PROF_PUT(d, 12, ps[1]); PROF_PUT(d, 13, ps[2]); PROF_PUT(d, 14, ps[3]); PROF_PUT(d, 15, ps[4]);
    (void)p_entries; (void)ps;
}

__global__ __launch_bounds__(TPB) void k_chunk_fold(Dev d)
{
    Ctrl *ctrl = d.ctrl;
    const uint32_t n = ctrl->chunk_ok;
    if (!ctrl->chunk_parallel || n == 0u) return;
    const uint32_t lane = threadIdx.x & 63u;
    const uint32_t wave = (blockIdx.x * TPB + threadIdx.x) >> 6, n_waves = (gridDim.x * TPB) >> 6;
    const uint32_t per_wave = ld(&ctrl->items_per_wave);
    if ((unsigned long long)per_wave * n_waves > d.items_cap) return;
    if (blockIdx.x == 0) {
        __shared__ uint32_t s_pref[CHUNK_WAVES_MAX + 1u];
        __shared__ uint32_t s_wtot[TPB / 64];
        const uint32_t pf0 = PROF_NOW();
        constexpr uint32_t RUN = CHUNK_WAVES_MAX / TPB;
        const uint32_t run = (n_waves + TPB - 1u) / TPB, b = threadIdx.x * run;
        uint32_t cnt[RUN];
        uint32_t sum = 0u;
#pragma unroll
        for (uint32_t k = 0; k < RUN; ++k) { cnt[k] = (k < run && b + k < n_waves) ? min(d.used_cnt[b + k], per_wave) : 0u; sum += cnt[k]; }
        uint32_t x = sum;
        for (uint32_t o = 1; o < 64u; o <<= 1) { const uint32_t y = __shfl_up(x, o, 64); if (lane >= o) x += y; }
        if (lane == 63u) s_wtot[threadIdx.x >> 6] = x;
        if (threadIdx.x == 0) s_pref[0] = 0u;
        __syncthreads();
        const uint32_t pf1 = PROF_NOW();
        uint32_t acc = x - sum;
        for (uint32_t k = 0; k < (threadIdx.x >> 6); ++k) acc += s_wtot[k];
#pragma unroll
        for (uint32_t k = 0; k < RUN; ++k) if (k < run && b + k < n_waves) { acc += cnt[k]; s_pref[b + k + 1u] = acc; }
        __syncthreads();
        const uint32_t pf2 = PROF_NOW();
        for (uint32_t w = threadIdx.x; w <= n_waves; w += TPB) d.used_pref[w] = s_pref[w];
        BOOKS_PROF(d, 8, pf1 - pf0); BOOKS_PROF(d, 9, pf2 - pf1); BOOKS_PROF(d, 10, PROF_NOW() - pf2);
        (void)pf0; (void)pf1; (void)pf2;
    }
    const uint32_t qr = wave & (SUBQ - 1u), first = wave >> 6, step = n_waves >> 6;
    const uint32_t n_list = step ? min(ld(&d.hot[(HOT_BIG + qr) * HOT_STRIDE]), d.big_qcap) : 0u;
#ifdef ESIM_PROFILE_FOLD
    const uint32_t pq0 = PROF_NOW();
    uint32_t pq_rec = 0u, pq_n = 0u;
    PROF_PUT(d, 11, 0u); PROF_PUT(d, 12, 0u); PROF_PUT(d, 13, 0u);
#endif
    if (first >= n_list) return;
    WORK_TALLY;
    const uint32_t *bl = d.big_list + (size_t)qr * d.big_qcap * 3u;
    const Decision q0 = lane < n ? d.dec[lane] : Decision{ 0u, 0u, 0u, 0u };
    const Decision q1 = 64u + lane < n ? d.dec[64u + lane] : Decision{ 0u, 0u, 0u, 0u };
    const M96 AW = { __ballot(lane < n && q0.at_work != 0u), (uint32_t)__ballot(64u + lane < n && q1.at_work != 0u) };
    const M96 BUS = { __ballot(lane < n && q0.bus_dir != 0u), (uint32_t)__ballot(64u + lane < n && q1.bus_dir != 0u) };
    for (uint32_t g = first; g < n_list; g += 64u * step) {
        uint32_t slot_l = 0u, base_l = 0u, n_ov_l = 0u, sch_l = 0xFFFFFFFFu;
        const uint32_t mine = g + lane * step;
        if (mine < n_list) {
            slot_l = bl[3u * mine]; base_l = bl[3u * mine + 1u];
            const uint32_t cap_l = bl[3u * mine + 2u] & 0x7FFFFFFFu, all_ovf = bl[3u * mine + 2u] >> 31;
            if (all_ovf) {
                sch_l = base_l; base_l = 0u;
                if (sch_l >= d.n_sch || slot_l >= d.hcap) { sch_l = 0xFFFFFFFFu; slot_l = 0u; RAISE(ctrl, ESIM_ERANGE, ERR_AT_BIG_LIST); }
            } else
            if (slot_l < d.hcap && base_l <= d.ovf_n && cap_l <= d.ovf_n - base_l) {
                const uint32_t state = d.slot_state[slot_l];
                n_ov_l = min((state > ITEM_RECS && state < SLOT_COUNTERS_ONLY) ? state - ITEM_RECS : 0u, cap_l);
            } else { slot_l = 0u; base_l = 0u; ctrl->error = (uint32_t)(-ESIM_ERANGE); }
        }
        const uint32_t m = min(64u, (n_list - g + step - 1u) / step);
        for (uint32_t i8 = 0; i8 < m; i8 += 8u) {
        uint32_t ivs[8];
#pragma unroll
        for (uint32_t u = 0; u < 8u; ++u) ivs[u] = (i8 + u < m && lane < FX(n_ov_l, min(i8 + u, 63u))) ? d.ovf[FX(base_l, min(i8 + u, 63u)) + lane] : 0u;
#pragma unroll
        for (uint32_t u = 0; u < 8u; ++u) {
            const uint32_t i = i8 + u;
            if (i >= m) break;
            const uint32_t slot = FX(slot_l, i), base = FX(base_l, i), n_ov = FX(n_ov_l, i);
            uint32_t iv = ivs[u];
            uint32_t c0 = 0u, c1 = 0u;
            WORK_ADD(WK_FOLDED, lane == 0 ? n_ov : 0);
            if (FX(sch_l, i) != 0xFFFFFFFFu) {
                uint32_t *dd = d.sch_diff + (size_t)FX(sch_l, i) * SD_REPL * 2u * FREE_MAX;
                uint32_t a0 = 0u, a1 = 0u, p0 = 0u, p1 = 0u;
#pragma unroll
                for (uint32_t r = 0; r < SD_REPL; ++r) {
                    uint32_t *rr = dd + (size_t)r * 2u * FREE_MAX;
                    a0 += rr[lane]; p0 += rr[FREE_MAX + lane];
                    if (lane < FREE_MAX - 64u) { a1 += rr[64u + lane]; p1 += rr[FREE_MAX + 64u + lane]; }
                }
#pragma unroll
                for (uint32_t r = 0; r < SD_REPL; ++r) {
                    uint32_t *rr = dd + (size_t)r * 2u * FREE_MAX;
                    rr[lane] = 0u; rr[FREE_MAX + lane] = 0u;
                    if (lane < FREE_MAX - 64u) { rr[64u + lane] = 0u; rr[FREE_MAX + 64u + lane] = 0u; }
                }
                for (uint32_t o = 1; o < 64u; o <<= 1) {
                    const uint32_t ya = __shfl_up(a0, o, 64), yp = __shfl_up(p0, o, 64), yb = __shfl_up(a1, o, 64), yq = __shfl_up(p1, o, 64);
                    if (lane >= o) { a0 += ya; p0 += yp; a1 += yb; p1 += yq; }
                }
                a1 += __shfl(a0, 63, 64); p1 += __shfl(p0, 63, 64);
                if (lane < n) c0 = ((AW.lo >> lane) & 1ull) ? a0 - (((BUS.lo >> lane) & 1ull) ? p0 : 0u) : 0u;
                if (lane < FREE_MAX - 64u && 64u + lane < n) c1 = ((AW.hi >> lane) & 1u) ? a1 - (((BUS.hi >> lane) & 1u) ? p1 : 0u) : 0u;
            }
#ifdef ESIM_PROFILE_FOLD
            pq_rec += n_ov; ++pq_n;
#endif
            for (uint32_t b = 0; b < n_ov; b += 64u) {
                if (b) iv = b + lane < n_ov ? d.ovf[base + b + lane] : 0u;
                const uint32_t nb = min(64u, n_ov - b);
                if (nb <= 12u) {
                    for (uint32_t k = 0; k < nb; ++k) {
                        iv_count(FX(iv, k), lane, AW, BUS, c0, c1);
                    }
                    continue;
                }
                const M96 at = iv_steps(iv, AW, BUS);
                for (uint32_t j = 0; j < n && j < 64u; ++j) {
                    const uint32_t k = (uint32_t)__popcll(__ballot((at.lo >> j) & 1ull));
                    if (lane == j) c0 += k;
                }
                for (uint32_t j = 64u; j < n; ++j) {
                    const uint32_t k = (uint32_t)__popcll(__ballot((at.hi >> (j - 64u)) & 1u));
                    if (lane == j - 64u) c1 += k;
                }
            }
            uint32_t *v = d.vec + (size_t)slot * FREE_MAX;
            if (lane < n && c0) atomicAdd(&v[lane], c0);
            if (64u + lane < n && c1) atomicAdd(&v[64u + lane], c1);
        }
        }
    }
    WORK_FLUSH(d);
#ifdef ESIM_PROFILE_FOLD
    PROF_PUT(d, 11, pq_n); PROF_PUT(d, 12, PROF_NOW() - pq0); PROF_PUT(d, 13, pq_rec);
#endif
}
```

Baseline: 58330 billion citizen-timesteps/s.

## Queue large member lists as units at mark time and process them in draw kernel

Large member lists are now split into fixed-member units when items are claimed in the marks kernel, instead of being split during the draw kernel. Those units are then drained at the start of k_chunk_draw using a software-pipelined prefetch, so k_chunk_units is left with only the big route pairs and is launched only when max_route exceeds 64. This removes a separate pass that had to wait for draw to finish, and sizes each unit by member count rather than by pairs. In exchange, marks does more serialized per-lane atomics and writes, and the draw kernel now requires its wave count to be a multiple of SUBQ.

```diff
diff --git a/epidemicsimulator_amd/csrc/esim_device.h b/epidemicsimulator_amd/csrc/esim_device.h
--- a/epidemicsimulator_amd/csrc/esim_device.h
+++ b/epidemicsimulator_amd/csrc/esim_device.h
@@ -101,6 +101,9 @@
 #define SD_REPL 8u
 
 struct ItemRec { uint32_t id, a_lo, a_hi, b_lo, b_hi, aux, link, own; };
+#define ITEM_INLINE_A 0x80000000u
+#define ITEM_INLINE_B 0x40000000u
+#define ITEM_AUX_MASK 0x3FFFFFFFu
 #define CHUNK_WAVES_MAX 4096u
 #define SLOT_COUNTERS_ONLY 0x40000000u
 #ifndef ITEM_RECS
@@ -241,10 +244,10 @@
 #define PAIR_K(per_wave, nbus) ((per_wave) * ((nbus) > 8u ? ((nbus) + 3u) / 4u : 2u))
 #define COUNT_GRID 256u
 #define EXP_ROWS 32u
-#ifndef UNIT_INLINE
-#define UNIT_INLINE 1024u
-#endif
 #ifndef UNIT_PAIRS
 #define UNIT_PAIRS 1024u
 #endif
+#define UNIT_SLOTS_MAX(n) (((n) + 3u) / 4u + 1u)
+#define UNIT_MEMBERS(n) (UNIT_PAIRS / UNIT_SLOTS_MAX(n))
+static_assert(UNIT_MEMBERS(FREE_MAX) >= 1u, "a unit holds at least one member over every slot of the longest chunk");
 #define CHUNK_ROUTE_MAX 2048u
diff --git a/epidemicsimulator_amd/csrc/esim_host_ctx.h b/epidemicsimulator_amd/csrc/esim_host_ctx.h
--- a/epidemicsimulator_amd/csrc/esim_host_ctx.h
+++ b/epidemicsimulator_amd/csrc/esim_host_ctx.h
@@ -115,7 +115,7 @@
     bool vax_repair_always = false;
     uint32_t tiny_pairs = 2048;
     uint32_t small_grid = 64, small_mult = 4;
-    uint32_t draw_mult = 4, units_mult = 4;
+    uint32_t draw_mult = 4;
     uint32_t small_max = 128;
     uint32_t pair_log2 = 0;
 };
diff --git a/epidemicsimulator_amd/csrc/esim_host_run.h b/epidemicsimulator_amd/csrc/esim_host_run.h
--- a/epidemicsimulator_amd/csrc/esim_host_run.h
+++ b/epidemicsimulator_amd/csrc/esim_host_run.h
@@ -153,11 +153,11 @@
     void front(bool few) const
     {
         const Tuning &t = c->tune;
-        const uint32_t g = few ? t.small_grid : t.grid_chunk, g_draw = g * (few ? t.small_mult : t.draw_mult), g_units = g * (few ? t.small_mult : t.units_mult);
+        const uint32_t g = few ? t.small_grid : t.grid_chunk, g_draw = g * (few ? t.small_mult : t.draw_mult);
         mark(ESIM_CK_MARKS); hipLaunchKernelGGL(k_chunk_marks, dim3(g), dim3(TPB), 0, c->stream, c->d);
         mark(ESIM_CK_FOLD); hipLaunchKernelGGL(k_chunk_fold, dim3(g), dim3(TPB), 0, c->stream, c->d);
         mark(ESIM_CK_DRAW); hipLaunchKernelGGL(k_chunk_draw, dim3(g_draw), dim3(TPB), 0, c->stream, c->d, g * (TPB / 64u));
-        mark(ESIM_CK_UNITS); hipLaunchKernelGGL(k_chunk_units, dim3(g_units), dim3(TPB), 0, c->stream, c->d);
+        if (c->d.max_route > 64u) { mark(ESIM_CK_UNITS); hipLaunchKernelGGL(k_chunk_units, dim3(g), dim3(TPB), 0, c->stream, c->d); }
     }
     void count() const { mark(ESIM_CK_COUNT); hipLaunchKernelGGL(k_chunk_count, dim3(COUNT_GRID), dim3(TPB), 0, c->stream, c->d); }
     void scatter() const { mark(ESIM_CK_SCATTER); hipLaunchKernelGGL(k_chunk_scatter, dim3(COUNT_GRID), dim3(TPB), 0, c->stream, c->d); }
diff --git a/epidemicsimulator_amd/csrc/esim_host_upload.h b/epidemicsimulator_amd/csrc/esim_host_upload.h
--- a/epidemicsimulator_amd/csrc/esim_host_upload.h
+++ b/epidemicsimulator_amd/csrc/esim_host_upload.h
@@ -192,14 +192,16 @@
     if ((rc = dev_alloc_fill(c, &d.slot_iv, (size_t)cap * SLOT_IV_STRIDE))) return rc;
     size_t units = 0;
     auto add_lists = [&](const std::vector<uint32_t> &off) {
+        const size_t M = UNIT_MEMBERS(FREE_MAX);
         for (size_t i = 0; i + 1 < off.size(); ++i) {
-            const size_t pairs = (size_t)(off[i + 1] - off[i]) * FREE_MAX;
-            if (pairs > UNIT_INLINE) units += (pairs + UNIT_PAIRS - 1) / UNIT_PAIRS;
+            const size_t n_mem = off[i + 1] - off[i];
+            if (n_mem > M) units += (n_mem + M - 1) / M;
         }
     };
     add_lists(u.res_off); add_lists(u.wrk_off); add_lists(u.room_off);
     units = std::min<size_t>(units, (size_t)N / 8u + 65536u);
     d.unit_qcap = (uint32_t)std::max<size_t>(1024, units * 2u / SUBQ);
+    if (const char *e = std::getenv("ESIM_UNIT_QCAP")) d.unit_qcap = (uint32_t)std::min<long>(1l << 24, std::max<long>(1, std::atol(e)));
     if ((rc = dev_alloc_fill(c, &d.units, (size_t)d.unit_qcap * SUBQ, 0xFF))) return rc;
     if ((rc = dev_alloc_fill(c, &d.route_pairs, (size_t)d.items_cap * (CHUNK_BUS_STEPS / 4u)))) return rc;
     d.big_pairs_cap = (uint32_t)std::max<size_t>(1, std::min<size_t>((size_t)d.items_cap / 4u, u.n_big_routes) * CHUNK_BUS_STEPS);
@@ -341,7 +343,6 @@
     if (const char *e = std::getenv("ESIM_SMALL_GRID")) t.small_grid = (uint32_t)std::max(0, std::atoi(e) / 16 * 16);
     if (const char *e = std::getenv("ESIM_SMALL_MULT")) t.small_mult = (uint32_t)std::min(16, std::max(1, std::atoi(e)));
     if (const char *e = std::getenv("ESIM_DRAW_MULT")) t.draw_mult = (uint32_t)std::min(4, std::max(1, std::atoi(e)));
-    if (const char *e = std::getenv("ESIM_UNITS_MULT")) t.units_mult = (uint32_t)std::min(16, std::max(1, std::atoi(e)));
     if (const char *e = std::getenv("ESIM_GRID_EXPOSE")) t.grid_expose = (uint32_t)std::max(1, std::atoi(e));
     t.pair_log2 = 0u;
     if (const char *e = std::getenv("ESIM_PAIR_LOG2")) t.pair_log2 = (uint32_t)std::min(31, std::max(6, std::atoi(e)));
diff --git a/epidemicsimulator_amd/csrc/esim_kernels_common.h b/epidemicsimulator_amd/csrc/esim_kernels_common.h
--- a/epidemicsimulator_amd/csrc/esim_kernels_common.h
+++ b/epidemicsimulator_amd/csrc/esim_kernels_common.h
@@ -129,6 +129,7 @@
        WK_RIDERS,
        WK_BUS_DRAWS,
        WK_HITS,
+       WK_UNIT_ROUNDS,
        WK_N };
 #define WORK_TALLY uint32_t wk_[WK_N]; for (int wk_i = 0; wk_i < WK_N; ++wk_i) wk_[wk_i] = 0u
 #define WORK_ADD(i, x) (wk_[i] += (uint32_t)(x))
diff --git a/epidemicsimulator_amd/csrc/esim_kernels_draw.h b/epidemicsimulator_amd/csrc/esim_kernels_draw.h
--- a/epidemicsimulator_amd/csrc/esim_kernels_draw.h
+++ b/epidemicsimulator_amd/csrc/esim_kernels_draw.h
@@ -157,29 +157,14 @@
     put_school(ws, lane, c0, c1);
 }
 
-struct UnitSrc { uint32_t slot, link, own; };
-__device__ __forceinline__ void list_or_units(const Dev &d, Ctrl *ctrl, const ChunkShared &sm, WaveScratch &ws, const uint32_t *idx,
-                                              uint32_t lo, uint32_t hi, const UnitSrc &src, uint32_t lane, uint32_t kind, uint32_t S, uint32_t t0 WORK_ARG,
-                                              bool have_pre = false, uint32_t pre_m = 0u, uint32_t pre_w = 0u)
+__device__ __forceinline__ bool list_with_item(uint32_t n_mem, uint32_t unit_m, uint32_t here) { return n_mem <= unit_m || here != 0u; }
+__device__ __forceinline__ void item_list(const Dev &d, Ctrl *ctrl, const ChunkShared &sm, WaveScratch &ws, const uint32_t *idx,
+                                          uint32_t lo, uint32_t hi, uint32_t unit_m, uint32_t here, uint32_t lane, uint32_t kind, uint32_t S, uint32_t t0 WORK_ARG,
+                                          uint32_t pre_m, uint32_t pre_w)
 {
     const uint32_t pairs = (hi - lo) * S;
-    if (pairs == 0) return;
-    if (pairs <= UNIT_INLINE) { member_pairs(d, ctrl, sm, ws, idx, lo, 0u, pairs, lane, kind, S, t0 WORK_PASS, have_pre, pre_m, pre_w); return; }
-    const uint32_t n_units = (pairs + UNIT_PAIRS - 1u) / UNIT_PAIRS;
-    const uint32_t r = ((blockIdx.x * TPB + threadIdx.x) >> 6) & (SUBQ - 1u);
-    uint32_t start = 0;
-    if (lane == 0) start = atomicAdd(&d.hot[(HOT_UNITS + r) * HOT_STRIDE], n_units);
-    start = __shfl(start, 0, 64);
-    UnitRec *q = d.units + (size_t)r * d.unit_qcap;
-    if (start + n_units > d.unit_qcap) {
-        for (uint32_t i = lane; i < n_units && start + i < d.unit_qcap; i += 64u) q[start + i].code = UNIT_NOOP;
-        member_pairs(d, ctrl, sm, ws, idx, lo, 0u, pairs, lane, kind, S, t0 WORK_PASS, have_pre, pre_m, pre_w);
-        return;
-    }
-    for (uint32_t i = lane; i < n_units; i += 64u) {
-        const uint32_t p_lo = i * UNIT_PAIRS;
-        q[start + i] = UnitRec{ src.slot, kind == 2u ? src.link : 0xFFFFFFFFu, lo, hi - lo, (kind << 30) | p_lo, src.own, p_lo / S, 0u };
-    }
+    if (pairs == 0 || !list_with_item(hi - lo, unit_m, here)) return;
+    member_pairs(d, ctrl, sm, ws, idx, lo, 0u, pairs, lane, kind, S, t0 WORK_PASS, true, pre_m, pre_w);
 }
 
 struct ItemFetch { uint32_t slot, id, a_lo, a_hi, b_lo, b_hi, aux, link, c0, c1; };
@@ -338,6 +323,29 @@
     __syncthreads();
 }
 
+__device__ __forceinline__ bool unit_ok(const Dev &d, uint32_t u)
+{
+    const uint32_t code = FX(u, 4), kind = code >> 30, m_cnt = code & 0x3FFFFFFFu, link = FX(u, 1), lo = FX(u, 2), n_mem = FX(u, 3), mf = FX(u, 6);
+    const unsigned long long end = (unsigned long long)lo + n_mem;
+    const bool fits = (kind == 0u && end <= d.n) | (kind == 1u && end <= d.n_wrk_idx) | (kind == 2u && end <= d.n_room_idx);
+    return fits && FX(u, 0) < d.hcap && (link == 0xFFFFFFFFu || link < d.hcap) && m_cnt != 0u && mf < n_mem && m_cnt <= n_mem - mf;
+}
+
+__device__ __forceinline__ void unit_stage2(const Dev &d, Ctrl *ctrl, uint32_t lane, uint32_t &u, uint32_t &xs, uint32_t &ys, uint32_t &mid)
+{
+    const uint32_t code = FX(u, 4);
+    if (code == UNIT_NOOP) return;
+    if (!unit_ok(d, u)) { if (lane == 0) RAISE(ctrl, ESIM_ERANGE, ERR_AT_ITEM_CHECK); u = 0xFFFFFFFFu; return; }
+    xs = fetch_slot(d, FX(u, 0), lane); ys = fetch_slot(d, FX(u, 1), lane);
+    const uint32_t kind = code >> 30, at = FX(u, 2) + FX(u, 6) + lane;
+    mid = at;
+    if (lane < (code & 0x3FFFFFFFu)) {
+        if (kind == 2u) mid = d.room_idx[at];
+        else if (kind == 1u) mid = d.wrk_idx[at];
+        else if (d.res_idx) mid = d.res_idx[at];
+    }
+}
+
 __global__ __launch_bounds__(TPB) void k_chunk_draw(Dev d, uint32_t n_mw)
 {
     __shared__ ChunkShared sm;
@@ -352,6 +360,7 @@
     uint32_t p_items = 0u, p_item_max = 0u;
     const uint32_t per_wave = ld(&ctrl->items_per_wave);
     if ((unsigned long long)per_wave * n_mw > d.items_cap || n_waves % n_mw != 0u) return;
+    if (n_waves % SUBQ != 0u) { if (lane == 0) ctrl->error = (uint32_t)(-ESIM_ERANGE); return; }
     const uint32_t G = n_waves / n_mw;
     const uint32_t T = d.used_pref[n_mw];
     const uint32_t coarse = d.used_pref[min(64u * lane, n_mw)];
@@ -389,16 +398,58 @@
     };
     auto deal_riders = [&]() { if (have) { const uint32_t r = code_l >> 7; off_l = d.route_off[r]; sz_l = d.route_off[r + 1] - off_l; } };
     deal(0u);
+    const uint32_t unit_m = UNIT_MEMBERS(min(n, FREE_MAX));
+    const uint32_t qr = wave & (SUBQ - 1u), u_first = wave / SUBQ, u_step = n_waves / SUBQ;
+    const uint32_t *q_words = reinterpret_cast<const uint32_t *>(d.units + (size_t)qr * d.unit_qcap);
+    const uint32_t n_units = min(ld(&d.hot[(HOT_UNITS + qr) * HOT_STRIDE]), d.unit_qcap);
+    auto unit_words = [&](uint32_t q) -> uint32_t { return lane < 8u ? q_words[(size_t)q * 8u + lane] : 0u; };
+    uint32_t u_0 = 0xFFFFFFFFu, u_1 = 0xFFFFFFFFu;
+    uint32_t xs_0 = 0u, ys_0 = 0u, mid_0 = 0u;
+    if (u_first < n_units) u_0 = unit_words(u_first);
+    if (u_first + u_step < n_units) u_1 = unit_words(u_first + u_step);
+    unit_stage2(d, ctrl, lane, u_0, xs_0, ys_0, mid_0);
     stage_chunk(d, sm, n, TPB);
     __syncthreads();
     const uint32_t route_base = d.n_bld + d.n_room;
-    WaveScratch &ws = wsc[threadIdx.x >> 6];
     const auto [AW, BUS, EV] = chunk_masks(sm.dec, lane, n);
     if (d_lo < d_hi) sl_cur = fetch_slot(d, FX(id_cur, LANE_HSLOT), lane);
     deal_riders();
+    WaveScratch &ws = wsc[threadIdx.x >> 6];
 #ifdef ESIM_WAVE_PROFILE
     if (lane == 0) ws.rounds = 0u;
 #endif
+    const uint32_t pu1 = PROF_NOW();
+    uint32_t pu_n = 0u, pu_max = 0u, pu_it = 0u;
+    for (uint32_t q = u_first; q < n_units; q += u_step) {
+        const uint32_t u = u_0, xs = xs_0, ys = ys_0, mid = mid_0;
+        u_0 = u_1;
+        u_1 = 0xFFFFFFFFu;
+        if (q + 2u * u_step < n_units) u_1 = unit_words(q + 2u * u_step);
+        if (q + u_step < n_units) unit_stage2(d, ctrl, lane, u_0, xs_0, ys_0, mid_0);
+        const uint32_t code = FX(u, 4);
+        if (code == UNIT_NOOP) continue;
+        const uint32_t pui = PROF_NOW();
+        ++pu_n;
+        const uint32_t kind = code >> 30, m_cnt = code & 0x3FFFFFFFu, slot = FX(u, 0), link = FX(u, 1), lo = FX(u, 2), own = FX(u, 5), mf = FX(u, 6);
+        const uint32_t mw = lane < m_cnt ? d.cit[mid] : 0u;
+        uint32_t c0, c1;
+        item_counts(d, xs, slot, lane, n, AW, BUS, c0, c1);
+        iv_count(own, lane, AW, BUS, c0, c1);
+        if (kind == 2u) {
+            uint32_t s0 = 0u, s1 = 0u;
+            if (link != 0xFFFFFFFFu) item_counts(d, ys, link, lane, n, AW, BUS, s0, s1);
+            put_school(ws, lane, s0, s1);
+        }
+        const uint32_t *idx = kind == 2u ? d.room_idx : kind == 1u ? d.wrk_idx : d.res_idx;
+        const uint32_t S = item_steps_regs(c0, c1, lane, ws, t0, AW, EV);
+        __builtin_amdgcn_wave_barrier();
+        if (S != 0u) {
+            WORK_ADD(WK_UNITS, lane == 0 ? 1 : 0); WORK_ADD(WK_UNIT_ROUNDS, lane == 0 ? (m_cnt * S + 63u) / 64u : 0);
+            member_pairs(d, ctrl, sm, ws, idx, lo, mf * S, (mf + m_cnt) * S, lane, kind, S, t0 WORK_PASS, true, mid, mw, mf);
+        }
+        __builtin_amdgcn_wave_barrier();
+        { const uint32_t dt = PROF_NOW() - pui; pu_max = dt > pu_max ? dt : pu_max; pu_it += (m_cnt * S + 63u) / 64u; }
+    }
     uint32_t pst[5] = { 0u, 0u, 0u, 0u, 0u };
     const uint32_t pt1 = PROF_NOW();
     for (uint32_t v = d_lo; v < d_hi; ++v) {
@@ -414,9 +465,12 @@
         const uint32_t pi0 = PROF_NOW();
         pst[0] += pi0 - pq0;
         (void)pi0; ++p_items; WORK_ADD(WK_ITEMS, lane == 0 ? 1 : 0);
+        const uint32_t here_a = it.aux & ITEM_INLINE_A, here_b = it.aux & ITEM_INLINE_B;
         if (it.id < d.n_bld) {
-            if (it.aux == ESIM_SCHOOL) continue;
-            const uint32_t n_res = it.a_hi - it.a_lo, n_wrk = it.b_hi - it.b_lo;
+            if ((it.aux & ITEM_AUX_MASK) == ESIM_SCHOOL) continue;
+            const uint32_t n_res = list_with_item(it.a_hi - it.a_lo, unit_m, here_a) ? it.a_hi - it.a_lo : 0u;
+            const uint32_t n_wrk = list_with_item(it.b_hi - it.b_lo, unit_m, here_b) ? it.b_hi - it.b_lo : 0u;
+            if ((n_res | n_wrk) == 0u) continue;
             uint32_t rm = 0u, wm = 0u, rw = 0u, ww = 0u;
             if (lane < n_res) rm = d.res_idx ? d.res_idx[it.a_lo + lane] : it.a_lo + lane;
             if (lane < n_wrk) wm = d.wrk_idx[it.b_lo + lane];
@@ -426,22 +480,21 @@
             const uint32_t S = item_steps_regs(it.c0, it.c1, lane, ws, t0, AW, EV);
             __builtin_amdgcn_wave_barrier();
             const uint32_t pq2 = PROF_NOW();
-            const UnitSrc src = { it.slot, it.link, FX(x, 7) };
-            list_or_units(d, ctrl, sm, ws, d.res_idx, it.a_lo, it.a_hi, src, lane, 0u, S, t0 WORK_PASS, true, rm, rw);
+            item_list(d, ctrl, sm, ws, d.res_idx, it.a_lo, it.a_lo + n_res, unit_m, here_a, lane, 0u, S, t0 WORK_PASS, rm, rw);
             const uint32_t pq3 = PROF_NOW();
-            list_or_units(d, ctrl, sm, ws, d.wrk_idx, it.b_lo, it.b_hi, src, lane, 1u, S, t0 WORK_PASS, true, wm, ww);
+            item_list(d, ctrl, sm, ws, d.wrk_idx, it.b_lo, it.b_lo + n_wrk, unit_m, here_b, lane, 1u, S, t0 WORK_PASS, wm, ww);
             const uint32_t pq4 = PROF_NOW();
             pst[1] += pq1 - pi0; pst[2] += pq2 - pq1; pst[3] += pq3 - pq2; pst[4] += pq4 - pq3;
         } else {
             const uint32_t n_mem = it.a_hi - it.a_lo;
+            if (!list_with_item(n_mem, unit_m, here_a)) continue;
             uint32_t mm = 0u, mw = 0u;
             if (lane < n_mem) mm = d.room_idx[it.a_lo + lane];
             school_counts(d, it.link, lane, n, ws);
             if (lane < n_mem) mw = d.cit[mm];
             const uint32_t S = item_steps_regs(it.c0, it.c1, lane, ws, t0, AW, EV);
             __builtin_amdgcn_wave_barrier();
-            const UnitSrc src = { it.slot, it.link, FX(x, 7) };
-            list_or_units(d, ctrl, sm, ws, d.room_idx, it.a_lo, it.a_hi, src, lane, 2u, S, t0 WORK_PASS, true, mm, mw);
+            item_list(d, ctrl, sm, ws, d.room_idx, it.a_lo, it.a_hi, unit_m, here_a, lane, 2u, S, t0 WORK_PASS, mm, mw);
         }
         __builtin_amdgcn_wave_barrier();
         { const uint32_t dt = PROF_NOW() - pi0; p_item_max = dt > p_item_max ? dt : p_item_max; }
@@ -461,83 +514,27 @@
     const uint32_t pt3 = PROF_NOW();
 #ifndef ESIM_PROFILE_UNITS
     PROF_PUT(d, 0, pt0); PROF_PUT(d, 1, pt1); PROF_PUT(d, 2, pt2); PROF_PUT(d, 3, pt3);
-    PROF_PUT(d, 4, p_items); PROF_PUT(d, 5, p_item_max); PROF_PUT(d, 6, wsc[threadIdx.x >> 6].rounds);
+    PROF_PUT(d, 4, p_items); PROF_PUT(d, 5, p_item_max); PROF_PUT(d, 6, ws.rounds);
     PROF_PUT(d, 11, pst[0]); PROF_PUT(d, 12, pst[1]); PROF_PUT(d, 13, pst[2]); PROF_PUT(d, 14, pst[3]); PROF_PUT(d, 15, pst[4]);
+#else
+    PROF_PUT(d, 0, pt0); PROF_PUT(d, 1, pu1); PROF_PUT(d, 2, pt1); PROF_PUT(d, 4, pu_n); PROF_PUT(d, 5, pu_max); PROF_PUT(d, 7, pu_it);
 #endif
-    (void)pst;
+    (void)pst; (void)pu1; (void)pu_n; (void)pu_max; (void)pu_it;
     (void)pt0; (void)pt1; (void)pt2; (void)pt3; (void)p_items; (void)p_item_max;
 }
 
 __global__ __launch_bounds__(TPB) void k_chunk_units(Dev d)
 {
     __shared__ ChunkShared sm;
-    __shared__ WaveScratch wsc[TPB / 64];
     __shared__ RouteShared rs;
     Ctrl *ctrl = d.ctrl;
     const uint32_t t0 = ctrl->chunk_t0, n = ctrl->chunk_ok;
     if (!ctrl->chunk_parallel || n == 0u) return;
-    const uint32_t lane = threadIdx.x & 63u;
-    const uint32_t wave = (blockIdx.x * TPB + threadIdx.x) >> 6, n_waves = (gridDim.x * TPB) >> 6;
-    const uint32_t pu0 = PROF_NOW();
+    const uint32_t n_pairs = min(ld(&d.hot[HOT_BIGPAIRS * HOT_STRIDE]), d.big_pairs_cap);
+    if (blockIdx.x >= n_pairs) return;
     WORK_TALLY;
-    uint32_t pu_n = 0u, pu_max = 0u, pu_it = 0u;
-    const uint32_t qr = wave & (SUBQ - 1u), first = wave / SUBQ, step = n_waves / SUBQ;
-    const uint32_t n_units = step ? min(ld(&d.hot[(HOT_UNITS + qr) * HOT_STRIDE]), d.unit_qcap) : 0u;
-    const uint32_t n_pairs = min(ld(&d.hot[HOT_BIGPAIRS * HOT_STRIDE]), d.big_pairs_cap);
-    if (__syncthreads_or(first < n_units) == 0 && n_pairs == 0u) return;
     stage_chunk(d, sm, n, TPB);
     __syncthreads();
-    WaveScratch &ws = wsc[threadIdx.x >> 6];
-    const uint32_t *q_words = reinterpret_cast<const uint32_t *>(d.units + (size_t)qr * d.unit_qcap);
-    const auto [AW, BUS, EV] = chunk_masks(sm.dec, lane, n);
-    auto unit_words = [&](uint32_t q) -> uint32_t { return lane < 8u ? q_words[(size_t)q * 8u + lane] : 0u; };
-    auto member_id = [&](uint32_t u) -> uint32_t {
-        const uint32_t code = FX(u, 4), kind = code >> 30, lo = FX(u, 2), n_mem = FX(u, 3), mf = FX(u, 6);
-        if (code == UNIT_NOOP || mf + lane >= n_mem) return 0u;
-        const uint32_t *idx = kind == 2u ? d.room_idx : kind == 1u ? d.wrk_idx : d.res_idx;
-        return idx ? idx[lo + mf + lane] : lo + mf + lane;
-    };
-    const uint32_t pu1 = PROF_NOW();
-    uint32_t u_0 = 0xFFFFFFFFu, u_1 = 0xFFFFFFFFu;
-    uint32_t xs_0 = 0u, ys_0 = 0u, mid_0 = 0u;
-    if (first < n_units) u_0 = unit_words(first);
-    if (first + step < n_units) u_1 = unit_words(first + step);
-    if (first < n_units && FX(u_0, 4) != UNIT_NOOP) { xs_0 = fetch_slot(d, FX(u_0, 0), lane); ys_0 = fetch_slot(d, FX(u_0, 1), lane); mid_0 = member_id(u_0); }
-    for (uint32_t q = first; q < n_units; q += step) {
-        const uint32_t u = u_0, xs = xs_0, ys = ys_0, mid = mid_0;
-        u_0 = u_1;
-        u_1 = 0xFFFFFFFFu;
-        if (q + 2u * step < n_units) u_1 = unit_words(q + 2u * step);
-        if (q + step < n_units && FX(u_0, 4) != UNIT_NOOP) { xs_0 = fetch_slot(d, FX(u_0, 0), lane); ys_0 = fetch_slot(d, FX(u_0, 1), lane); mid_0 = member_id(u_0); }
-        const uint32_t code = FX(u, 4);
-        if (code == UNIT_NOOP) continue;
-        const uint32_t pui = PROF_NOW();
-        ++pu_n;
-        const uint32_t kind = code >> 30, p_lo = code & 0x3FFFFFFFu, slot = FX(u, 0), link = FX(u, 1), lo = FX(u, 2), n_mem = FX(u, 3), own = FX(u, 5), mf = FX(u, 6);
-        const uint32_t mw = (mf + lane < n_mem) ? d.cit[mid] : 0u;
-        uint32_t c0, c1;
-        item_counts(d, xs, slot, lane, n, AW, BUS, c0, c1);
-        iv_count(own, lane, AW, BUS, c0, c1);
-        if (kind == 2u) {
-            uint32_t s0 = 0u, s1 = 0u;
-            if (link != 0xFFFFFFFFu) item_counts(d, ys, link, lane, n, AW, BUS, s0, s1);
-            put_school(ws, lane, s0, s1);
-        }
-        const uint32_t *idx = kind == 2u ? d.room_idx : kind == 1u ? d.wrk_idx : d.res_idx;
-        const uint32_t S = item_steps_regs(c0, c1, lane, ws, t0, AW, EV);
-        __builtin_amdgcn_wave_barrier();
-        const uint32_t pairs = n_mem * S;
-        WORK_ADD(WK_UNITS, lane == 0 ? 1 : 0);
-        member_pairs(d, ctrl, sm, ws, idx, lo, p_lo, min(pairs, p_lo + UNIT_PAIRS), lane, kind, S, t0 WORK_PASS, true, mid, mw, mf);
-        __builtin_amdgcn_wave_barrier();
-        { const uint32_t dt = PROF_NOW() - pui; pu_max = dt > pu_max ? dt : pu_max; pu_it += (min(pairs, p_lo + UNIT_PAIRS) - p_lo + 63u) / 64u; }
-    }
-    const uint32_t pu2 = PROF_NOW();
-    WORK_FLUSH(d);
-#ifdef ESIM_PROFILE_UNITS
-    PROF_PUT(d, 0, pu0); PROF_PUT(d, 1, pu1); PROF_PUT(d, 2, pu2); PROF_PUT(d, 4, pu_n); PROF_PUT(d, 5, pu_max); PROF_PUT(d, 7, pu_it);
-#endif
-    (void)pu0; (void)pu1; (void)pu2; (void)pu_n; (void)pu_max; (void)pu_it;
     for (uint32_t q = blockIdx.x; q < n_pairs; q += gridDim.x) route_pair_big<TPB>(d, ctrl, sm, rs, d.route_pairs_big[q], t0, n WORK_PASS);
     WORK_FLUSH(d);
 }
diff --git a/epidemicsimulator_amd/csrc/esim_kernels_marks.h b/epidemicsimulator_amd/csrc/esim_kernels_marks.h
--- a/epidemicsimulator_amd/csrc/esim_kernels_marks.h
+++ b/epidemicsimulator_amd/csrc/esim_kernels_marks.h
@@ -8,6 +8,22 @@
 }
 
 #define ITEM_UNUSED 0xFFFFFFFFu
+
+__device__ __forceinline__ bool queue_units(const Dev &d, uint32_t r, uint32_t M, uint32_t kind, uint32_t slot, uint32_t link, uint32_t lo,
+                                            uint32_t hi, uint32_t own)
+{
+    if (hi <= lo || hi - lo <= M) return true;
+    const uint32_t n_mem = hi - lo, n_units = (n_mem + M - 1u) / M;
+    const uint32_t start = atomicAdd(&d.hot[(HOT_UNITS + r) * HOT_STRIDE], n_units);
+    UnitRec *q = d.units + (size_t)r * d.unit_qcap;
+    if (start >= d.unit_qcap || n_units > d.unit_qcap - start) {
+        for (uint32_t i = start; i < d.unit_qcap && i - start < n_units; ++i) q[i].code = UNIT_NOOP;
+        return false;
+    }
+    for (uint32_t i = 0; i < n_units; ++i)
+        q[start + i] = UnitRec{ slot, link, lo, n_mem, (kind << 30) | min(M, n_mem - i * M), own, i * M, 0u };
+    return true;
+}
 
 __global__ __launch_bounds__(TPB) void k_chunk_marks(Dev d)
 {
@@ -24,6 +40,7 @@
     if (wave == 0 && lane == 0) { ctrl->items_per_wave = per_wave; ctrl->n_items = per_wave * n_waves; }
     if ((unsigned long long)per_wave * n_waves > d.items_cap) { if (lane == 0) ctrl->error = (uint32_t)(-ESIM_ERANGE); return; }
     uint32_t next_id = wave * per_wave;
+    const uint32_t unit_q = wave & (SUBQ - 1u), unit_m = UNIT_MEMBERS(min(n, FREE_MAX));
     const ChunkMasks cm = chunk_masks(d.dec, lane, n);
     const M96 &AW = cm.AW, &BUS = cm.BUS;
     const unsigned long long lt = (1ull << lane) - 1ull;
@@ -128,11 +145,16 @@
                 if (k == 0u || k == 1u) {
                     const uint4 b4 = *reinterpret_cast<const uint4 *>(&d.bld8[id]);
                     rec.a_lo = b4.x; rec.a_hi = b4.y; rec.b_lo = b4.z; rec.b_hi = b4.w;
-                    rec.aux = d.bld8[id].type;
+                    rec.aux = d.bld8[id].type & ITEM_AUX_MASK;
+                    if (rec.aux != ESIM_SCHOOL) {
+                        if (!queue_units(d, unit_q, unit_m, 0u, slot[k], 0xFFFFFFFFu, rec.a_lo, rec.a_hi, rec.own)) rec.aux |= ITEM_INLINE_A;
+                        if (!queue_units(d, unit_q, unit_m, 1u, slot[k], 0xFFFFFFFFu, rec.b_lo, rec.b_hi, rec.own)) rec.aux |= ITEM_INLINE_B;
+                    }
                 } else if (k == 2u) {
                     const uint32_t r = id - d.n_bld;
                     rec.a_lo = d.room_off[r]; rec.a_hi = d.room_off[r + 1u];
-                    rec.aux = d.room_bld[r];
+                    rec.aux = d.room_bld[r] & ITEM_AUX_MASK;
+                    if (!queue_units(d, unit_q, unit_m, 2u, slot[k], rec.link, rec.a_lo, rec.a_hi, rec.own)) rec.aux |= ITEM_INLINE_A;
                 }
                 d.item_rec[v] = rec;
             }
```

Result: slower. 57020 billion citizen-timesteps/s (-2.2%).
